# intellerce/controlanimate

Hardware: AMD Instinct MI355X
Metric: frames_per_sec (higher is better)
Workload: dtype fp16

## Files before the change

### controlanimate_amd/_capi.py

```python
from __future__ import annotations

import ctypes as C
import os

_HERE = os.path.dirname(os.path.abspath(__file__))
LIB_PATH = os.environ.get("CA_HIP_LIB") or os.path.join(_HERE, "csrc", "libcontrolanimate_hip.so")

CA_BF16, CA_F16 = 0, 1
CA_F32 = 2
CA_ACT_NONE, CA_ACT_SILU = 0, 1
CA_ACT_RELU = 4
CA_ACT_RELU6 = 5
CA_ACT_LEAKY02 = 6
CA_MLSD_TOPK = 200
CA_POSE_MAX_PEAKS, CA_POSE_MAX_PEOPLE, CA_POSE_AREA_TAPS = 64, 64, 8
CA_POSE_OVERFLOW_PEAKS, CA_POSE_OVERFLOW_PEOPLE = 1, 2
CA_POSE_OVERFLOW_FACES, CA_POSE_OVERFLOW_FACE_RESIZE = 4, 8
CA_FACE_SIZE, CA_FACE_HEAT, CA_FACE_PARTS, CA_FACE_MIN_SIDE, CA_FACE_SLOT_INTS = 384, 48, 71, 11, 8
CA_FACE_MODE_NONE, CA_FACE_MODE_LANCZOS4, CA_FACE_MODE_AREA = 0, 1, 2
CA_POSE_OVERFLOW_HANDS, CA_POSE_OVERFLOW_HAND_RESIZE = 16, 32
CA_HAND_PARTS, CA_HAND_HEAT_COLS, CA_HAND_MAP, CA_HAND_SCALES, CA_HAND_SLOT_INTS = 21, 24, 128, 4, 8
CA_HAND_MODE_NONE, CA_HAND_MODE_RESIZE, CA_HAND_MIN_BOX, CA_HAND_AREA_TAPS = 0, 1, 20, 16
ABI_VERSION = 16


class CAHipUnavailable(RuntimeError):
    pass


class CAHipError(RuntimeError):
    pass


class GemmArgs(C.Structure):
    _fields_ = [
        ("a", C.c_void_p), ("a2", C.c_void_p), ("w", C.c_void_p), ("c", C.c_void_p),
        ("bias", C.c_void_p), ("rowbias", C.c_void_p), ("residual", C.c_void_p),
        ("lda", C.c_int64), ("lda2", C.c_int64), ("ldc", C.c_int64), ("ld_res", C.c_int64),
        ("ld_rowbias", C.c_int64),
        ("m", C.c_int32), ("n", C.c_int32), ("k1", C.c_int32), ("k2", C.c_int32),
        ("rows_per_group", C.c_int32),
        ("alpha", C.c_float), ("post_scale", C.c_float),
        ("act", C.c_int32), ("geglu", C.c_int32), ("out_f32", C.c_int32), ("dtype", C.c_int32),
        ("ln_stats", C.c_void_p), ("ln_colsum", C.c_void_p), ("ln_eps", C.c_float),
        ("workspace", C.c_void_p), ("workspace_bytes", C.c_int64),
        ("row_sums_out", C.c_void_p), ("ln_parts", C.c_int32),
        ("w_frag", C.c_void_p),
    ]


class FfArgs(C.Structure):
    _fields_ = [
        ("x", C.c_void_p), ("w1_frag", C.c_void_p), ("bias1", C.c_void_p), ("colsum1", C.c_void_p), ("ln_stats", C.c_void_p),
        ("w2_frag", C.c_void_p), ("bias2", C.c_void_p), ("residual", C.c_void_p), ("y", C.c_void_p),
        ("lda", C.c_int64), ("ldc", C.c_int64), ("ld_res", C.c_int64),
        ("m", C.c_int32), ("c", C.c_int32), ("inner", C.c_int32), ("ln_eps", C.c_float), ("dtype", C.c_int32),
        ("w_out_frag", C.c_void_p), ("bias_out", C.c_void_p), ("residual_out", C.c_void_p), ("ld_res_out", C.c_int64),
    ]


class TattnArgs(C.Structure):
    _fields_ = [
        ("x", C.c_void_p), ("w_frag", C.c_void_p), ("gamma", C.c_void_p), ("bias_pe", C.c_void_p), ("o", C.c_void_p),
        ("lda", C.c_int64), ("ldo", C.c_int64), ("ld_bias_pe", C.c_int64),
        ("batch", C.c_int32), ("frames", C.c_int32), ("tokens", C.c_int32), ("heads", C.c_int32), ("c", C.c_int32),
        ("ln_eps", C.c_float), ("scale", C.c_float), ("dtype", C.c_int32),
        ("w_out_frag", C.c_void_p), ("bias_out", C.c_void_p), ("residual", C.c_void_p), ("ld_res", C.c_int64),
    ]


ATTN_WOUT_FRAG_ELEMS = 102400
TATTN_W_FRAG_ELEMS = 368640


class XattnArgs(C.Structure):
    _fields_ = [
        ("x", C.c_void_p), ("wq_frag", C.c_void_p), ("bias", C.c_void_p), ("kv_frag", C.c_void_p), ("o", C.c_void_p),
        ("lda", C.c_int64), ("ldo", C.c_int64),
        ("m", C.c_int32), ("tokens", C.c_int32), ("frames_per_kv", C.c_int32), ("kv_mod", C.c_int32), ("kv_batches", C.c_int32),
        ("nk", C.c_int32), ("heads", C.c_int32), ("c", C.c_int32),
        ("ln_eps", C.c_float), ("dtype", C.c_int32),
        ("w_out_frag", C.c_void_p), ("bias_out", C.c_void_p), ("residual", C.c_void_p), ("ld_res", C.c_int64),
        ("kv_frag_ip", C.c_void_p), ("nk_ip", C.c_int32), ("ip_scale", C.c_float),
    ]


XATTN_W_FRAG_ELEMS = 122880
XATTN_KV_FRAG_ELEMS = 7680


class ConvArgs(C.Structure):
    _fields_ = [
        ("x", C.c_void_p), ("x2", C.c_void_p), ("w", C.c_void_p), ("y", C.c_void_p),
        ("bias", C.c_void_p), ("rowbias", C.c_void_p), ("residual", C.c_void_p),
        ("ld_res", C.c_int64), ("ld_rowbias", C.c_int64),
        ("images", C.c_int32), ("hin", C.c_int32), ("win", C.c_int32),
        ("cin1", C.c_int32), ("cin2", C.c_int32), ("cout", C.c_int32),
        ("stride", C.c_int32), ("upsample", C.c_int32), ("rows_per_group", C.c_int32),
        ("alpha", C.c_float), ("post_scale", C.c_float),
        ("act", C.c_int32), ("out_f32", C.c_int32), ("dtype", C.c_int32),
# ... 49 lines not shown
    ]


class PerceiverAttnArgs(C.Structure):
    _fields_ = [
        ("q", C.c_void_p), ("x", C.c_void_p), ("l", C.c_void_p), ("o", C.c_void_p),
        ("q_row", C.c_int64), ("q_batch", C.c_int64),
        ("x_row", C.c_int64), ("x_batch", C.c_int64), ("x_v_off", C.c_int64),
        ("l_row", C.c_int64), ("l_batch", C.c_int64), ("l_v_off", C.c_int64),
        ("o_row", C.c_int64), ("o_batch", C.c_int64),
        ("batches", C.c_int32), ("heads", C.c_int32), ("head_dim", C.c_int32),
        ("nq", C.c_int32), ("n_x", C.c_int32), ("n_l", C.c_int32),
        ("scale", C.c_float), ("dtype", C.c_int32),
    ]


class ModconvArgs(C.Structure):
    _fields_ = [
        ("x", C.c_void_p), ("wt", C.c_void_p), ("s", C.c_void_p), ("demod", C.c_void_p), ("noise", C.c_void_p), ("bias", C.c_void_p),
        ("sft_scale", C.c_void_p), ("sft_shift", C.c_void_p), ("y", C.c_void_p),
        ("s_stride", C.c_int64), ("demod_stride", C.c_int64),
        ("images", C.c_int32), ("h", C.c_int32), ("w", C.c_int32), ("cin", C.c_int32), ("cout", C.c_int32),
        ("upsample", C.c_int32), ("x_shared", C.c_int32),
        ("noise_weight", C.c_float), ("dtype", C.c_int32),
    ]


class Conv7x7Args(C.Structure):
    _fields_ = [
        ("x", C.c_void_p * 2), ("w", C.c_void_p * 2), ("bias", C.c_void_p * 2), ("y", C.c_void_p * 2),
        ("ldx", C.c_int64), ("ldy", C.c_int64),
        ("groups", C.c_int32), ("images", C.c_int32), ("h", C.c_int32), ("w_px", C.c_int32), ("cin", C.c_int32), ("cout", C.c_int32),
        ("relu", C.c_int32), ("dtype", C.c_int32),
    ]


SYMBOLS = {
    "ca_abi_version": (C.c_int, []),
    "ca_last_error": (C.c_char_p, []),
    "ca_gemm": (C.c_int, [C.POINTER(GemmArgs), C.c_void_p]),
    "ca_pack_w_frag": (C.c_int, [C.c_void_p, C.c_int32, C.c_int32, C.c_int32, C.c_void_p, C.c_void_p]),
    "ca_pack_w2_frag": (C.c_int, [C.c_void_p, C.c_int32, C.c_int32, C.c_void_p, C.c_void_p]),
    "ca_ff_fused": (C.c_int, [C.POINTER(FfArgs), C.c_void_p]),
    "ca_ff_fused_supported": (C.c_int, [C.POINTER(FfArgs)]),
    "ca_tattn_fused": (C.c_int, [C.POINTER(TattnArgs), C.c_void_p]),
    "ca_tattn_fused_supported": (C.c_int, [C.POINTER(TattnArgs)]),
    "ca_pack_w_tattn": (C.c_int, [C.c_void_p, C.c_int32, C.c_int32, C.c_void_p, C.c_void_p]),
    "ca_pack_w_out": (C.c_int, [C.c_void_p, C.c_int32, C.c_int32, C.c_void_p, C.c_void_p]),
    "ca_xattn_fused": (C.c_int, [C.POINTER(XattnArgs), C.c_void_p]),
    "ca_xattn_fused_supported": (C.c_int, [C.POINTER(XattnArgs)]),
    "ca_xattn_pack_w": (C.c_int, [C.c_void_p, C.c_int32, C.c_int32, C.c_void_p, C.c_void_p]),
    "ca_xattn_pack_kv": (C.c_int, [C.c_void_p, C.c_int64, C.c_int32, C.c_int32, C.c_int32, C.c_int32, C.c_float, C.c_int32, C.c_void_p, C.c_void_p]),
    "ca_gemm_ln_inline_supported": (C.c_int, [C.POINTER(GemmArgs)]),
    "ca_gemm_wants_finished_stats": (C.c_int, [C.POINTER(GemmArgs)]),
    "ca_ln_finish_sums": (C.c_int, [C.c_void_p, C.c_int, C.c_int64, C.c_int, C.c_float, C.c_void_p, C.c_void_p]),
    "ca_gemm_workspace_bytes": (C.c_int64, [C.POINTER(GemmArgs)]),
    "ca_gemm_row_sums_parts": (C.c_int, [C.POINTER(GemmArgs)]),
    "ca_gemm_plan_name": (C.c_int, [C.POINTER(GemmArgs), C.c_char_p, C.c_int32]),
    "ca_conv3x3_plan_name": (C.c_int, [C.POINTER(ConvArgs), C.c_char_p, C.c_int32]),
    "ca_conv3x3": (C.c_int, [C.POINTER(ConvArgs), C.c_void_p]),
    "ca_pack_w_wino": (C.c_int, [C.c_void_p, C.c_int32, C.c_int32, C.c_int32, C.c_void_p, C.c_void_p]),
    "ca_conv3x3_workspace_bytes": (C.c_int64, [C.POINTER(ConvArgs)]),
    "ca_softmax_rows": (C.c_int, [C.c_void_p, C.c_void_p, C.c_int64, C.c_int32, C.c_int64, C.c_int64, C.c_float, C.c_int32, C.c_void_p]),
    "ca_groupnorm_partials_floats": (C.c_int64, [C.c_int32, C.c_int32, C.c_int32, C.c_int32]),
    "ca_groupnorm_stats": (C.c_int, [C.POINTER(GroupNormArgs), C.c_void_p]),
    "ca_groupnorm_apply": (C.c_int, [C.POINTER(GroupNormArgs), C.c_void_p]),
    "ca_groupnorm": (C.c_int, [C.POINTER(GroupNormArgs), C.c_void_p]),
    "ca_groupnorm_wino_supported": (C.c_int, [C.POINTER(GroupNormArgs)]),
    "ca_layernorm": (C.c_int, [C.POINTER(LayerNormArgs), C.c_void_p]),
    "ca_attention": (C.c_int, [C.POINTER(AttnArgs), C.c_void_p]),
    "ca_attention_plan_name": (C.c_int, [C.POINTER(AttnArgs), C.c_char_p, C.c_int32]),
    "ca_add_bcast": (C.c_int, [C.c_void_p, C.c_void_p, C.c_void_p, C.c_int64, C.c_int64, C.c_int32, C.c_void_p]),
    "ca_repeat": (C.c_int, [C.c_void_p, C.c_void_p, C.c_int64, C.c_int32, C.c_void_p]),
    "ca_silu_f32": (C.c_int, [C.c_void_p, C.c_void_p, C.c_int64, C.c_void_p]),
    "ca_timestep_embedding": (C.c_int, [C.c_void_p, C.c_float, C.c_void_p, C.c_int32, C.c_int32, C.c_int32, C.c_void_p]),
    "ca_latents_to_nhwc": (C.c_int, [C.c_void_p, C.c_void_p, C.c_int32, C.c_int32, C.c_int32, C.c_int32, C.c_int32,
                                      C.c_int32, C.c_int32, C.c_float, C.c_int32, C.c_void_p]),
    "ca_nhwc_to_ncfhw_f32": (C.c_int, [C.c_void_p, C.c_void_p, C.c_int32, C.c_int32, C.c_int32, C.c_int32, C.c_int32,
                                        C.c_int32, C.c_int32, C.c_int32, C.c_void_p]),
    "ca_ncfhw_to_nhwc": (C.c_int, [C.c_void_p, C.c_int32, C.POINTER(C.c_int64), C.c_void_p, C.c_int32, C.c_int32,
                                    C.c_int32, C.c_int32, C.c_int32, C.c_int32, C.c_int32, C.c_void_p]),
    "ca_cfg_scheduler_step": (C.c_int, [C.c_void_p, C.c_int32, C.c_int32, C.c_float, C.c_void_p, C.c_void_p,
                                         C.c_void_p, C.c_void_p, C.c_int32, C.c_int32, C.c_int32, C.c_int32,
                                         C.POINTER(C.c_float), C.c_float, C.c_void_p]),
    "ca_lincomb": (C.c_int, [C.c_void_p, C.POINTER(C.c_void_p), C.POINTER(C.c_float), C.c_int32, C.c_int64, C.c_void_p]),
    "ca_conv3x3_narrow": (C.c_int, [C.POINTER(ConvNarrowArgs), C.c_void_p]),
    "ca_conv3x3_narrow_plan_name": (C.c_int, [C.POINTER(ConvNarrowArgs), C.c_char_p, C.c_int32]),
    "ca_rgb8_to_nhwc": (C.c_int, [C.c_void_p, C.c_void_p, C.c_int32, C.c_int32, C.c_int32, C.c_int32, C.c_void_p]),
    "ca_resize_lanczos4_u8": (C.c_int, [C.c_void_p, C.c_void_p, C.c_int32, C.c_int32, C.c_int32, C.c_int32, C.c_int32,
                                         C.c_void_p, C.c_void_p, C.c_void_p, C.c_void_p, C.c_void_p]),
    "ca_color_match_workspace_bytes": (C.c_int64, [C.c_int32, C.c_int64]),
    "ca_hist_u8x3": (C.c_int, [C.c_void_p, C.c_void_p, C.c_int32, C.c_int64, C.c_void_p]),
    "ca_color_moments_f64": (C.c_int, [C.c_void_p, C.c_void_p, C.c_void_p, C.c_void_p, C.c_int32, C.c_int64, C.c_void_p, C.c_int64, C.c_void_p]),
    "ca_color_transform_f64": (C.c_int, [C.c_void_p, C.c_void_p, C.c_void_p, C.c_void_p, C.c_void_p, C.c_void_p, C.c_int32, C.c_int64, C.c_void_p]),
    "ca_sort_f64_segments": (C.c_int, [C.c_void_p, C.c_void_p, C.c_int32, C.c_int64, C.c_void_p, C.c_int64, C.c_void_p]),
    "ca_color_rank_map_f64": (C.c_int, [C.c_void_p, C.c_void_p, C.c_void_p, C.c_void_p, C.c_void_p, C.c_void_p, C.c_int32, C.c_int64,
                                         C.c_void_p, C.c_int64, C.c_void_p]),
    "ca_color_finish_u8": (C.c_int, [C.c_void_p, C.c_void_p, C.c_int32, C.c_int64, C.c_int32, C.c_void_p, C.c_int64, C.c_void_p]),
    "ca_canny_workspace_bytes": (C.c_int64, [C.c_int32, C.c_int32, C.c_int32]),
    "ca_canny_tile_w": (C.c_int32, []),
    "ca_canny_tile_h": (C.c_int32, []),
    "ca_canny_classify": (C.c_int, [C.c_void_p, C.c_int32, C.c_int32, C.c_int32, C.c_int32, C.c_int32, C.c_int32, C.c_void_p, C.c_int64, C.c_void_p]),
    "ca_canny_link": (C.c_int, [C.c_int32, C.c_int32, C.c_int32, C.c_void_p, C.c_int64, C.c_void_p]),
    "ca_canny_link_stage": (C.c_int, [C.c_int32, C.c_int32, C.c_int32, C.c_void_p, C.c_int64, C.c_int32, C.c_void_p]),
    "ca_canny_emit": (C.c_int, [C.c_int32, C.c_int32, C.c_int32, C.c_void_p, C.c_int64, C.c_void_p, C.c_void_p, C.c_int32, C.c_int32, C.c_void_p]),
    "ca_conv_up2_phase_supported": (C.c_int, [C.POINTER(ConvArgs)]),
# ... 106 lines not shown
```

### controlanimate_amd/context.py

```python
from __future__ import annotations

from dataclasses import dataclass, field
from typing import Optional

import torch


@dataclass
class ExecCtx:
    b: int
    f: int
    dtype: torch.dtype
    temb: torch.Tensor
    emb_groups: int
    ehs: Optional[torch.Tensor] = None
    frames_per_kv: int = 1
    kv_mod: int = 0
    gn_frames_per_stat: int = 1
    cache: dict = field(default_factory=dict)

    @property
    def images(self) -> int:
        return self.b * self.f

    def rows_per_emb_group(self, h: int, w: int) -> int:
        return self.images // self.emb_groups * h * w


class Dispatch:
    gemm_ar = True
    ff_fused = True
    tattn_fused = True
    xattn_fused = True
    attn_out_fused = True
    xattn_ip_fused = True
    conv_winograd = True
    gn_winograd = True
    conv_up2_phase = True
    ln_row_sums = True
    repeat_kernel = True
    ln_fold = True
    cfg_shared = True
    cn_cfg_dedup = True
    pdc_block_fused = True
    dpt_head_fused = False
    pose_conv7_direct = True
    controlnet_streams = 2


dispatch = Dispatch()
```

### controlanimate_amd/controlnet.py

```python
from __future__ import annotations

import dataclasses
from collections import OrderedDict

from typing import List, Optional, Sequence, Tuple, Union

import torch
from torch import nn

from . import kernels as K
from .context import ExecCtx
from .layers import HipConv1x1, HipConv3x3
from .unet import FrozenConfig, HipModelMixin, TimestepEmbedding, Timesteps
from .unet_blocks import UNetMidBlock3DCrossAttn, get_down_block


class ControlNetConditioningEmbedding(nn.Module):
    def __init__(self, conditioning_embedding_channels: int, conditioning_channels: int = 3,
                 block_out_channels: Tuple[int, ...] = (16, 32, 96, 256)):
        super().__init__()
        self.conv_in = HipConv3x3(conditioning_channels, block_out_channels[0])
        blocks = []
        for i in range(len(block_out_channels) - 1):
            blocks.append(HipConv3x3(block_out_channels[i], block_out_channels[i]))
# ... 136 lines not shown
    def residual_scales(self, conditioning_scale: float, guess_mode: bool) -> List[float]:
        n = len(self.controlnet_down_blocks) + 1
        if guess_mode:
            return [float(s) * conditioning_scale for s in torch.logspace(-1, 0, n)]
        return [float(conditioning_scale)] * n

    @torch.no_grad()
    def forward_body(self, x: torch.Tensor, timestep, encoder_hidden_states: torch.Tensor, controlnet_cond: torch.Tensor,
                     conditioning_scale: float = 1.0, guess_mode: bool = False, cfg_identical_halves: bool = False):
        device = x.device
        self._ensure_ready(device)
        images = x.shape[0]
        ehs, cache = self._prompt(encoder_hidden_states, device)
        nb = ehs.shape[0]
        temb = self._time_embedding(timestep, 1, device)
        ctx = ExecCtx(b=images, f=1, dtype=self.act_dtype, temb=temb, emb_groups=1, ehs=ehs, frames_per_kv=1, kv_mod=nb,
                      gn_frames_per_stat=1, cache=cache)
        hint_ent = self._hint(controlnet_cond, device)
        hint = hint_ent["emb"]
        if hint.shape[0] != images:
            raise ValueError(f"controlnet_cond batch {hint.shape[0]} != sample batch {images}")
        first = self.down_blocks[0]
        from .context import dispatch
        same_inputs = (cfg_identical_halves and images % 2 == 0 and bool(hint_ent["doubled"]) and
                       (not torch.is_tensor(timestep) or timestep.numel() == 1))
        if same_inputs and dispatch.cn_cfg_dedup and (images // 2) % nb == 0:
            half = images // 2
            hctx = dataclasses.replace(ctx, b=half)
            x = self.conv_in.run(x[:half], residual=hint[:half])
            outs = [x]
            for blk in self.down_blocks:
                x, o = blk(x, hctx)
                outs += o
            x = self.mid_block(x, hctx)
            return outs, x, self.residual_scales(conditioning_scale, guess_mode), True
        shared = same_inputs and dispatch.cfg_shared and getattr(first, "has_cross_attention", False)
        if shared:
            half = images // 2
            xh = self.conv_in.run(x[:half], residual=hint[:half])
            outs = [K.repeat_batch(xh)]
            x, o = first(xh, ctx, half_ctx=dataclasses.replace(ctx, b=half))
            outs += o
        else:
            x = self.conv_in.run(x, residual=hint)
            outs = [x]
        for blk in (self.down_blocks[1:] if shared else self.down_blocks):
            x, o = blk(x, ctx)
            outs += o
        x = self.mid_block(x, ctx)
        return outs, x, self.residual_scales(conditioning_scale, guess_mode), False

    @torch.no_grad()
    def apply_zero_convs(self, outs, x, scales, accumulate: Optional[Tuple[List[torch.Tensor], torch.Tensor]] = None, twice: bool = False):
        def one(zc, o, scale, prev):
            B_, h, w, c = o.shape
            rows = B_ * h * w
            a = o.view(rows, c)
            if not twice:
                return zc.run(a, alpha=scale, residual=None if prev is None else prev.view(rows, c)).view(B_, h, w, c)
            full = torch.empty((2 * B_, h, w, c), device=o.device, dtype=o.dtype)
            for hf in range(2):
                zc.run(a, alpha=scale, residual=None if prev is None else prev.view(2 * rows, c)[hf * rows:(hf + 1) * rows],
                       out=full.view(2 * rows, c)[hf * rows:(hf + 1) * rows])
            return full
        down = [one(zc, o, scales[i], None if accumulate is None else accumulate[0][i])
                for i, (zc, o) in enumerate(zip(self.controlnet_down_blocks, outs))]
        mid = one(self.controlnet_mid_block, x, scales[-1], None if accumulate is None else accumulate[1])
        return down, mid

    @torch.no_grad()
    def forward_nhwc(self, x: torch.Tensor, timestep, encoder_hidden_states: torch.Tensor, controlnet_cond: torch.Tensor,
                     conditioning_scale: float = 1.0, guess_mode: bool = False,
                     accumulate: Optional[Tuple[List[torch.Tensor], torch.Tensor]] = None, cfg_identical_halves: bool = False):
        outs, xm, scales, twice = self.forward_body(x, timestep, encoder_hidden_states, controlnet_cond, conditioning_scale, guess_mode,
                                                    cfg_identical_halves)
        return self.apply_zero_convs(outs, xm, scales, accumulate, twice)

    def forward(self, sample: torch.Tensor, timestep, encoder_hidden_states: torch.Tensor, controlnet_cond: torch.Tensor,
                conditioning_scale: float = 1.0, class_labels=None, timestep_cond=None, attention_mask=None,
                cross_attention_kwargs=None, guess_mode: bool = False, return_dict: bool = False):
        if not sample.is_cuda:
            raise RuntimeError("ControlNetModel runs on the HIP device only (no CPU fallback)")
        self._ensure_ready(sample.device)
        x = K.ncfhw_to_nhwc(sample.unsqueeze(2), self.conv_in.cin_pad, self.act_dtype)
        down, mid = self.forward_nhwc(x, timestep, encoder_hidden_states, controlnet_cond, conditioning_scale, guess_mode)
        return tuple(d.permute(0, 3, 1, 2) for d in down), mid.permute(0, 3, 1, 2)


class MultiControlNetModel(nn.Module):

    def __init__(self, controlnets: Sequence[ControlNetModel]):
        super().__init__()
        self.nets = nn.ModuleList(controlnets)

    @property
    def dtype(self):
        return self.nets[0].dtype

    def half(self):
        for n in self.nets:
            n.half()
        return self

    def prepare(self, device=None, dtype=None):
        for n in self.nets:
            n.prepare(device, dtype)
        return self

    def forward_bodies(self, x, timestep, encoder_hidden_states, controlnet_cond: Sequence[torch.Tensor],
                       conditioning_scale: Sequence[float], guess_mode: bool = False, cfg_identical_halves: bool = False, streams=None):
        bodies = []
        for i, (net, cond, scale) in enumerate(zip(self.nets, controlnet_cond, conditioning_scale)):
            if streams:
# ... 28 lines not shown
```

### controlanimate_amd/csrc/ca_gemm.hip

```cpp

#include "ca_gemm_plan.h"

namespace {
using namespace ca_gemm_detail;
#include "ca_conv_wino.h"

template <int DT, int BM, int BN, int WAVES_M, int WAVES_N, int MODE>
__global__ __launch_bounds__(256) void k_gemm(GemmKParams p) {
  constexpr int TM = BM / WAVES_M / 16;
  constexpr int TN = BN / WAVES_N / 16;
  constexpr int AI = BM / 32;
  constexpr int BI = BN / 32;
  static_assert(2 * (BM + BN) * BK >= BM * (BN + 8), "epilogue staging must fit");
  __shared__ __attribute__((aligned(16))) u16 smem[2 * (BM + BN) * BK];

  const int tid = threadIdx.x;
  const int lane = tid & 63;
  const int wid = tid >> 6;
  const int wm = wid / WAVES_N, wn = wid % WAVES_N;
  const int g = lane >> 4, l15 = lane & 15;

  const int tiles_n = (p.n + BN - 1) / BN;
  const unsigned bid = xcd_remap(blockIdx.x, gridDim.x);
  int tile_m, tile_n;
// ... 64 lines not shown
    } else {
      const int64_t ld = src2 ? p.lda2 : p.lda;
#pragma unroll
      for (int i = 0; i < AI; ++i) {
        ra[i] = (cok && a_ok[i]) ? ld16(base + a_rowoff[i] * ld + cio) : zero4;
      }
    }
  };
  auto store_tile = [&](int buf) {
    u16* sa = smem + buf * (BM + BN) * BK;
    u16* sb = sa + BM * BK;
#pragma unroll
    for (int i = 0; i < AI; ++i) st16(sa + lds_off(lr + 32 * i, lc), ra[i]);
#pragma unroll
    for (int i = 0; i < BI; ++i) st16(sb + lds_off(lr + 32 * i, lc), rb[i]);
  };

  f32x4 acc[TM][TN];
#pragma unroll
  for (int i = 0; i < TM; ++i)
#pragma unroll
    for (int j = 0; j < TN; ++j) acc[i][j] = (f32x4){0.f, 0.f, 0.f, 0.f};

  const int nt = p.taps * p.kc_tiles;
  load_tile(0);
  store_tile(0);
  __syncthreads();

  for (int t = 0; t < nt; ++t) {
    const int buf = t & 1;
    if (t + 1 < nt) load_tile(t + 1);
    const u16* sa = smem + buf * (BM + BN) * BK;
    const u16* sb = sa + BM * BK;
#pragma unroll
    for (int s = 0; s < 2; ++s) {
      u32x4 fa[TM], fb[TN];
#pragma unroll
      for (int i = 0; i < TM; ++i) fa[i] = ld16(sa + lds_off(wm * TM * 16 + i * 16 + l15, s * 4 + g));
#pragma unroll
      for (int j = 0; j < TN; ++j) fb[j] = ld16(sb + lds_off(wn * TN * 16 + j * 16 + l15, s * 4 + g));
#pragma unroll
      for (int i = 0; i < TM; ++i)
#pragma unroll
        for (int j = 0; j < TN; ++j) acc[i][j] = Elem<DT>::mfma(fb[j], fa[i], acc[i][j]);
    }
    if (t + 1 < nt) store_tile(buf ^ 1);
    __syncthreads();
  }

  gemm_epilogue<DT, BM, BN, TM, TN>(p, acc, smem, m0, n0, wm, wn, l15, g, tid);
}


template <int DT, int BM, int BN, int WAVES_M, int WAVES_N, int MODE, int NBUF>
__global__ __launch_bounds__(256, NBUF == 1 ? (BN > 128 ? 3 : 4) : 2)
void k_gemm_dma(GemmKParams p) {
  static_assert(WAVES_M * WAVES_N == 4 && (NBUF == 1 || NBUF == 3), "instantiations: see above");
  constexpr int KT = BK;
  constexpr int CPR = KT / 8;
  constexpr int RPI = 64 / CPR;
  constexpr int NW = WAVES_M * WAVES_N, NT = NW * 64;
  constexpr int TM = BM / WAVES_M / 16;
  constexpr int TN = BN / WAVES_N / 16;
  constexpr int AG = BM / RPI / NW;
  constexpr int BG = BN / RPI / NW;
  constexpr int SMEM_ELEMS = NBUF * (BM + BN) * KT > BM * (BN + 8) ? NBUF * (BM + BN) * KT : BM * (BN + 8);
  auto swz = [](int row) { return (row >> 1) & 7; };
  auto lds_at = [&](int row, int chunk) { return row * KT + ((chunk ^ swz(row)) << 3); };
  __shared__ __attribute__((aligned(16))) u16 smem[SMEM_ELEMS];

  const int tid = threadIdx.x;
  const int lane = tid & 63;
  const int wid = tid >> 6;
  const int wm = wid / WAVES_N, wn = wid % WAVES_N;
  const int g = lane >> 4, l15 = lane & 15;

  const int tiles_n = (p.n + BN - 1) / BN;
  const int tiles_m = (p.m + BM - 1) / BM;
  unsigned bid = xcd_remap(blockIdx.x, gridDim.x);
  int split = 0;
  if (p.splits > 1) {
    split = bid / (unsigned)(tiles_m * tiles_n);
    bid -= split * (unsigned)(tiles_m * tiles_n);
  }
  int tile_m, tile_n;
  tile_coords(bid, tiles_m, tiles_n, tile_m, tile_n);
  const int m0 = tile_m * BM, n0 = tile_n * BN;

  const __amdgpu_buffer_rsrc_t rs_a = __builtin_amdgcn_make_buffer_rsrc((void*)p.a, 0, p.a_bytes, 0x00020000);
  const __amdgpu_buffer_rsrc_t rs_a2 = __builtin_amdgcn_make_buffer_rsrc((void*)(p.a2 ? p.a2 : p.a), 0, p.a2 ? p.a2_bytes : p.a_bytes, 0x00020000);
  const __amdgpu_buffer_rsrc_t rs_w = __builtin_amdgcn_make_buffer_rsrc((void*)p.w, 0, p.w_bytes, 0x00020000);

  const int r8 = lane / CPR, cp = lane % CPR;
  const int kc = p.c1 + p.c2;
  const int kct = kc / KT;
  const unsigned wld = (unsigned)(p.taps * kc);

  int a_chunk[AG], a_img[AG], a_ho[AG], a_wo[AG];
  unsigned a_off1[AG], a_off2[AG];
  bool a_ok[AG];
#pragma unroll
  for (int i = 0; i < AG; ++i) {
    const int row = (wid * AG + i) * RPI + r8;
    a_chunk[i] = cp ^ swz(row);
    const int m = m0 + row;
    a_ok[i] = m < p.m;
    const int mm = a_ok[i] ? m : p.m - 1;
// ... 78 lines not shown
#pragma unroll
      for (int i = 0; i < TM; ++i) fa[i] = ld16(sa + lds_at(wm * TM * 16 + i * 16 + l15, s * 4 + g));
#pragma unroll
      for (int j = 0; j < TN; ++j) fb[j] = ld16(sb + lds_at(wn * TN * 16 + j * 16 + l15, s * 4 + g));
#pragma unroll
      for (int i = 0; i < TM; ++i)
#pragma unroll
        for (int j = 0; j < TN; ++j) acc[i][j] = Elem<DT>::mfma(fb[j], fa[i], acc[i][j]);
    }
  };
  if (NBUF == 1) {
    for (int t = 0; t < nt; ++t) {
      stage(t_first + t, 0);
      __syncthreads();
      compute(0);
      __syncthreads();
    }
  } else {
    constexpr int PER = AG + BG;
    static_assert((NBUF - 2) * PER < 64, "vmcnt");
#pragma unroll
    for (int s = 0; s < NBUF - 1; ++s)
      if (s < nt) stage(t_first + s, s);
    int slot = 0, slot_in = NBUF - 1;
    for (int t = 0; t < nt; ++t) {
      const int younger = nt - 1 - t < NBUF - 2 ? nt - 1 - t : NBUF - 2;
      if (younger <= 0) asm volatile("s_waitcnt vmcnt(0)" ::: "memory");
      else if (younger == 1) asm volatile("s_waitcnt vmcnt(%0)" ::"n"(PER) : "memory");
      else if (younger == 2) asm volatile("s_waitcnt vmcnt(%0)" ::"n"(2 * PER) : "memory");
      else asm volatile("s_waitcnt vmcnt(%0)" ::"n"((NBUF - 2) * PER < 64 ? (NBUF - 2) * PER : 0) : "memory");
      __builtin_amdgcn_s_barrier();
      if (t + NBUF - 1 < nt) stage(t_first + t + NBUF - 1, slot_in);
      compute(slot);
      asm volatile("s_waitcnt lgkmcnt(0)" ::: "memory");
      slot = slot + 1 == NBUF ? 0 : slot + 1;
      slot_in = slot_in + 1 == NBUF ? 0 : slot_in + 1;
    }
    __syncthreads();
  }
  if (p.splits > 1) {
    float* slab = p.partial + (int64_t)split * p.m * p.n;
#pragma unroll
    for (int i = 0; i < TM; ++i) {
      const int m = m0 + wm * TM * 16 + i * 16 + l15;
      if (m >= p.m) continue;
#pragma unroll
      for (int j = 0; j < TN; ++j) {
        const int n = n0 + wn * TN * 16 + j * 16 + g * 4;
        if (n < p.n) *reinterpret_cast<f32x4*>(slab + (int64_t)m * p.n + n) = acc[i][j];
      }
    }
    return;
  }
  gemm_epilogue<DT, BM, BN, TM, TN, NT>(p, acc, smem, m0, n0, wm, wn, l15, g, tid);
}

template <int DT>
__global__ __launch_bounds__(256) void k_splitk_reduce(GemmKParams p) {
  const int64_t id = (int64_t)blockIdx.x * 256 + threadIdx.x;
  const int c8n = p.n >> 3;
  const int64_t m = id / c8n;
  if (m >= p.m) return;
  const int n = (int)(id - m * c8n) * 8;
  float v[8];
#pragma unroll
  for (int k = 0; k < 8; ++k) v[k] = 0.f;
  for (int sp = 0; sp < p.splits; ++sp) {
    const float* src = p.partial + ((int64_t)sp * p.m + m) * p.n + n;
    const f32x4 a = *reinterpret_cast<const f32x4*>(src), b = *reinterpret_cast<const f32x4*>(src + 4);
#pragma unroll
    for (int k = 0; k < 4; ++k) {
      v[k] += a[k];
      v[4 + k] += b[k];
    }
  }
  if (p.ln_stats) {
    const float2 st = *reinterpret_cast<const float2*>(p.ln_stats + m * 2);
#pragma unroll
    for (int k = 0; k < 8; ++k) v[k] = st.y * (v[k] - st.x * p.ln_colsum[n + k]);
  }
  if (p.bias) {
#pragma unroll
    for (int k = 0; k < 8; ++k) v[k] += p.bias[n + k];
  }
  if (p.rowbias) {
    const float* rbp = p.rowbias + (m / p.rows_per_group) * p.ld_rowbias + n;
#pragma unroll
    for (int k = 0; k < 8; ++k) v[k] += rbp[k];
  }
#pragma unroll
  for (int k = 0; k < 8; ++k) v[k] *= p.alpha;
  unpack8<DT>(pack8<DT>(v), v);
  if (p.res) {
    float r[8];
    unpack8<DT>(ld16(p.res + m * p.ld_res + n), r);
#pragma unroll
    for (int k = 0; k < 8; ++k) v[k] += r[k];
  }
#pragma unroll
  for (int k = 0; k < 8; ++k) v[k] *= p.post;
  if (p.act != CA_ACT_NONE) {
#pragma unroll
    for (int k = 0; k < 8; ++k) v[k] = act_f(v[k], p.act);
  }
  const int64_t off = m * p.ldc + n;
  if (p.out_f32) {
    float* cp = reinterpret_cast<float*>(p.c) + off;
    *reinterpret_cast<f32x4*>(cp) = (f32x4){v[0], v[1], v[2], v[3]};
    *reinterpret_cast<f32x4*>(cp + 4) = (f32x4){v[4], v[5], v[6], v[7]};
  } else {
    st16(reinterpret_cast<u16*>(p.c) + off, pack8<DT>(v));
  }
}

template <int DT, int MODE>
int launch_gemm(const GemmKParams& p, const GemmPlan& g, hipStream_t st) {
  const dim3 grid(ceil_div_i(p.m, g.bm) * ceil_div_i(p.n, g.bn));
  switch (g.kind) {
    case PK_WRES: return ca_launch_gemm_pp(p, DT, MODE, PK_WRES, 0u, st);
    case PK_AR: return ca_launch_gemm_ar(p, DT, st);
    case PK_PP2:
    case PK_PS:
    case PK_PQ: return ca_launch_gemm_pp(p, DT, MODE, g.kind, g.tiles, st);
    case PK_PP2_SPLITK: {
      GemmKParams q = p;
      q.splits = g.splits;
      const int rc = ca_launch_gemm_pp(q, DT, MODE, PK_PP2, g.tiles * (unsigned)g.splits, st);
      hipLaunchKernelGGL((k_splitk_reduce<DT>), dim3(ceil_div_i((int64_t)q.m * (q.n / 8), 256)), dim3(256), 0, st, q);
      return rc;
    }
    case PK_DMA_SPLITK:
      hipLaunchKernelGGL((k_gemm_dma<DT, 128, 128, 2, 2, MODE, 1>), dim3(g.tiles * (unsigned)p.splits), dim3(256), 0, st, p);
      hipLaunchKernelGGL((k_splitk_reduce<DT>), dim3(ceil_div_i((int64_t)p.m * (p.n / 8), 256)), dim3(256), 0, st, p);
      return CA_OK;
    case PK_DMA:
      if (g.bn == 160 && g.nbuf == 1) hipLaunchKernelGGL((k_gemm_dma<DT, 128, 160, 2, 2, MODE, 1>), grid, dim3(256), 0, st, p);
      else if (g.bn == 128 && g.nbuf == 1) hipLaunchKernelGGL((k_gemm_dma<DT, 128, 128, 2, 2, MODE, 1>), grid, dim3(256), 0, st, p);
      else if (g.bn == 64 && g.nbuf == 1) hipLaunchKernelGGL((k_gemm_dma<DT, 128, 64, 4, 1, MODE, 1>), grid, dim3(256), 0, st, p);
      else if (g.bn == 64 && g.nbuf == 3) hipLaunchKernelGGL((k_gemm_dma<DT, 128, 64, 4, 1, MODE, 3>), grid, dim3(256), 0, st, p);
      else break;
      return CA_OK;
    case PK_REG:
      if (g.bn == 128) hipLaunchKernelGGL((k_gemm<DT, 128, 128, 2, 2, MODE>), grid, dim3(256), 0, st, p);
      else if (g.bn == 64) hipLaunchKernelGGL((k_gemm<DT, 128, 64, 4, 1, MODE>), grid, dim3(256), 0, st, p);
      else break;
      return CA_OK;
  }
  CA_FAIL(CA_ERR_LAUNCH, "ca_gemm: no kernel for plan kind %d, tile %dx%d, %d stages", (int)g.kind, g.bm, g.bn, g.nbuf);
}

}

extern "C" int ca_gemm(const ca_gemm_args* a, void* stream) {
  DenseLaunch d;
  int rc = gemm_prepare(a, d);
  if (rc) return rc;
  hipStream_t st = (hipStream_t)stream;
  rc = a->dtype == CA_BF16 ? launch_gemm<CA_BF16, 0>(d.p, d.plan, st) : launch_gemm<CA_F16, 0>(d.p, d.plan, st);
  if (rc) return rc;
  CA_CHECK_LAUNCH("ca_gemm");
  return CA_OK;
}

extern "C" int64_t ca_gemm_workspace_bytes(const ca_gemm_args* a) {
  DenseLaunch d;
  return gemm_resolve(a, d) == CA_OK ? d.workspace : 0;
}

extern "C" int ca_gemm_row_sums_parts(const ca_gemm_args* a) {
  DenseLaunch d;
  DenseAsk ask{};
  ask.without_row_sums = true;
  return gemm_resolve(a, d, ask) == CA_OK ? row_sums_parts_of(d.p) : 0;
}

extern "C" int ca_gemm_ln_inline_supported(const ca_gemm_args* a) {
  DenseLaunch d;
  return a && a->ln_colsum && gemm_resolve(a, d) == CA_OK && wres_eligible(d.p) ? 1 : 0;
}

extern "C" int ca_gemm_wants_finished_stats(const ca_gemm_args* a) {
  if (!a || !a->ln_colsum || !a->ln_stats || a->ln_parts <= 0 || a->row_sums_out) return 0;
  DenseLaunch d;
  DenseAsk ask{};
  ask.stats_finished = true;
  return gemm_resolve(a, d, ask) == CA_OK && d.plan.kind == PK_PQ ? 1 : 0;
}

extern "C" int64_t ca_conv3x3_workspace_bytes(const ca_conv_args* a) { return conv_workspace_bytes(a); }

static int launch_conv_wino(const ca_conv_args* a, const GemmKParams& cp, hipStream_t st) {
  const int kc = a->cin1 + a->cin2;
  const ConvGeom g = conv_geom(a);
  const int64_t tiles = wino_tiles(a, g);
  WinoParams w{};
  w.x = (const u16*)a->x;
  w.x2 = (const u16*)a->x2;
  w.v = (u16*)a->workspace;
  u16* mm = (u16*)a->workspace + (a->x_is_wino_v ? 0 : 16 * tiles * kc);
  w.mm = mm;
  w.y = (u16*)a->y;
  w.bias = a->bias;
  w.rowbias = a->rowbias;
  w.res = (const u16*)a->residual;
  w.ld_res = a->ld_res;
  w.ld_rowbias = a->ld_rowbias;
  w.images = a->images, w.h = g.hl, w.w = g.wl, w.c1 = a->cin1, w.c2 = a->cin2, w.cout = a->cout;
  w.ups = a->upsample;
  w.rows_per_group = cp.rows_per_group;
  w.alpha = a->alpha, w.post = a->post_scale, w.act = a->act;
  const int64_t in_threads = tiles * (kc / 8), out_threads = tiles * (a->cout / 8);
  if (a->x_is_wino_v) w.v = (u16*)a->x;
  else if (a->dtype == CA_BF16) hipLaunchKernelGGL((k_wino_in<CA_BF16>), dim3((unsigned)((in_threads + 255) / 256)), dim3(256), 0, st, w);
  else hipLaunchKernelGGL((k_wino_in<CA_F16>), dim3((unsigned)((in_threads + 255) / 256)), dim3(256), 0, st, w);
  GemmKParams q{};
  q.a = w.v;
  q.w = (const u16*)a->w_wino;
  q.c = mm;
  q.lda = kc;
  q.ldc = a->cout;
  q.a_bytes = desc_bytes(16 * tiles * kc);
  q.w_bytes = desc_bytes((int64_t)16 * a->cout * kc);
  q.m = (int)(16 * tiles);
  q.n = a->cout;
  q.c1 = kc;
  q.taps = 1;
// ... 89 lines not shown
```

### controlanimate_amd/csrc/ca_gemm_core.h

```cpp
#pragma once
#include "ca_common.h"
#include <stdlib.h>

namespace ca_gemm_detail {


struct GemmKParams {
  const u16* a;
  const u16* a2;
  const u16* w;
  void* c;
  const float* bias;
  const float* rowbias;
  const float* ln_stats;
  const float* ln_colsum;
  const u16* res;
  int64_t lda, lda2, ldc, ld_res, ld_rowbias;
  unsigned a_bytes, a2_bytes, w_bytes;
  int m, n;
  int c1, c2;
  int taps;
  int kc_tiles;
  int hin, win, hout, wout, stride, ups, pad_lo;
  int rows_per_group;
  float alpha, post;
  int act, geglu, out_f32;
  int splits;
  float* partial;
  int dbg;
  int tap_inner;
  float* row_sums;
  int ln_parts;
  int ln_inline;
  float ln_eps;
  const u16* wf;
  int w_group_rows;
  unsigned w_group_stride;
  int up2_rows, up2_tiles;
  unsigned up2_mag_w, up2_mag_h;
};

constexpr int BK = 64;

constexpr int GROUP_M = 8;
__device__ __forceinline__ void tile_coords(unsigned bid, int tiles_m, int tiles_n, int& tile_m, int& tile_n) {
  const unsigned gsz = GROUP_M * tiles_n;
  const unsigned group = bid / gsz, in = bid - group * gsz;
  const int first_m = group * GROUP_M;
  const int gm = tiles_m - first_m < GROUP_M ? tiles_m - first_m : GROUP_M;
  tile_m = first_m + in % gm;
  tile_n = in / gm;
}

__device__ __forceinline__ void k_tile_split(const GemmKParams& p, int t, int kct, int& tap, int& cc) {
  if (p.taps == 1) {
    tap = 0;
    cc = t;
  } else if (p.tap_inner) {
    cc = t / p.taps;
    tap = t - cc * p.taps;
  } else {
    tap = t / kct;
    cc = t - tap * kct;
  }
}

__device__ __forceinline__ int lds_off(int row, int chunk) {
  return row * BK + ((chunk ^ ((row >> 1) & 7)) << 3);
}

template <int DT, int TM, int TN>
__device__ __forceinline__ void gemm_epilogue_direct(const GemmKParams& p, f32x4 (&acc)[TM][TN], int m0, int n0, int wm, int wn,
                                                     int l15, int g) {
#pragma unroll
  for (int i = 0; i < TM; ++i) {
    const int m = m0 + wm * TM * 16 + i * 16 + l15;
    if (m >= p.m) continue;
    const float* rbp = p.rowbias ? p.rowbias + (int64_t)(m / p.rows_per_group) * p.ld_rowbias : nullptr;
#pragma unroll
    for (int j = 0; j < TN; ++j) {
      const int n = n0 + wn * TN * 16 + j * 16 + g * 4;
      if (n >= p.n) continue;
      float v[4];
#pragma unroll
      for (int r = 0; r < 4; ++r) v[r] = acc[i][j][r];
      if (p.bias) {
        f32x4 b = *reinterpret_cast<const f32x4*>(p.bias + n);
#pragma unroll
        for (int r = 0; r < 4; ++r) v[r] += b[r];
      }
      if (rbp) {
        f32x4 b = *reinterpret_cast<const f32x4*>(rbp + n);
#pragma unroll
        for (int r = 0; r < 4; ++r) v[r] += b[r];
      }
#pragma unroll
      for (int r = 0; r < 4; ++r) v[r] *= p.alpha;
      if (p.res) {
        u32x2 rr = *reinterpret_cast<const u32x2*>(p.res + (int64_t)m * p.ld_res + n);
        v[0] += Elem<DT>::to_f((u16)(rr[0] & 0xffffu));
        v[1] += Elem<DT>::to_f((u16)(rr[0] >> 16));
        v[2] += Elem<DT>::to_f((u16)(rr[1] & 0xffffu));
        v[3] += Elem<DT>::to_f((u16)(rr[1] >> 16));
      }
#pragma unroll
      for (int r = 0; r < 4; ++r) v[r] *= p.post;
      if (p.act != CA_ACT_NONE) {
#pragma unroll
        for (int r = 0; r < 4; ++r) v[r] = act_f(v[r], p.act);
      }
      if (p.geglu) {
        const f32x2 gg = gelu_erf_f2((f32x2){v[1], v[3]});
        float o0 = v[0] * gg[0];
        float o1 = v[2] * gg[1];
        const int64_t off = (int64_t)m * p.ldc + (n >> 1);
        if (p.out_f32) {
          float* cp = reinterpret_cast<float*>(p.c) + off;
          cp[0] = o0;
          cp[1] = o1;
        } else {
          *reinterpret_cast<unsigned*>(reinterpret_cast<u16*>(p.c) + off) = pack2<DT>(o0, o1);
        }
      } else {
        const int64_t off = (int64_t)m * p.ldc + n;
        if (p.out_f32) {
          *reinterpret_cast<f32x4*>(reinterpret_cast<float*>(p.c) + off) = (f32x4){v[0], v[1], v[2], v[3]};
        } else {
          u32x2 o;
          o[0] = pack2<DT>(v[0], v[1]);
          o[1] = pack2<DT>(v[2], v[3]);
          *reinterpret_cast<u32x2*>(reinterpret_cast<u16*>(p.c) + off) = o;
        }
      }
    }
  }
}

template <int DT, int BM, int BN, int TM, int TN, int NT = 256, bool ROWSUM = false>
__device__ __forceinline__ void gemm_epilogue(const GemmKParams& p, f32x4 (&acc)[TM][TN], u16* cs, int m0, int n0, int wm, int wn,
                                              int l15, int g, int tid, float2* rs = nullptr) {
  if (p.n < 8) {
    gemm_epilogue_direct<DT, TM, TN>(p, acc, m0, n0, wm, wn, l15, g);
    return;
  }
  constexpr int CLD = BN + 8;
  float2 ln_st[TM];
  f32x4 ln_cs[TN];
  if (p.ln_stats) {
#pragma unroll
    for (int i = 0; i < TM; ++i) {
      const int m = m0 + wm * TM * 16 + i * 16 + l15;
      if (p.ln_parts > 0) {
        float a = 0.f, b = 0.f;
        if (m < p.m) {
          for (int q = 0; q < p.ln_parts; ++q) {
            const float2 v = *reinterpret_cast<const float2*>(p.ln_stats + ((int64_t)m * p.ln_parts + q) * 2);
            a += v.x;
            b += v.y;
          }
        }
        const float inv = 1.f / (float)(p.c1 + p.c2);
        const float mean = a * inv;
        ln_st[i] = make_float2(mean, rsqrtf(fmaxf(b * inv - mean * mean, 0.f) + p.ln_eps));
      } else {
        ln_st[i] = m < p.m ? *reinterpret_cast<const float2*>(p.ln_stats + (int64_t)m * 2) : make_float2(0.f, 0.f);
      }
    }
#pragma unroll
    for (int j = 0; j < TN; ++j) {
      const int n = n0 + wn * TN * 16 + j * 16 + g * 4;
      ln_cs[j] = n < p.n ? *reinterpret_cast<const f32x4*>(p.ln_colsum + n) : (f32x4){0.f, 0.f, 0.f, 0.f};
    }
  }
  f32x4 rb_q[TN];
  bool rb_uniform = false;
  if (p.rowbias) {
    const int r_first = m0 + wm * TM * 16, r_last = r_first + TM * 16 - 1;
    rb_uniform = r_last < p.m && r_first / p.rows_per_group == r_last / p.rows_per_group;
    if (rb_uniform) {
      const float* base = p.rowbias + (int64_t)(r_first / p.rows_per_group) * p.ld_rowbias;
#pragma unroll
      for (int j = 0; j < TN; ++j) {
        const int n = n0 + wn * TN * 16 + j * 16 + g * 4;
        rb_q[j] = n < p.n ? *reinterpret_cast<const f32x4*>(base + n) : (f32x4){0.f, 0.f, 0.f, 0.f};
      }
    }
  }
#pragma unroll
  for (int i = 0; i < TM; ++i) {
    const int row = wm * TM * 16 + i * 16 + l15;
    const int m = m0 + row;
    const float* rbp = (p.rowbias && !rb_uniform && m < p.m) ? p.rowbias + (int64_t)(m / p.rows_per_group) * p.ld_rowbias : nullptr;
#pragma unroll
    for (int j = 0; j < TN; ++j) {
      const int col = wn * TN * 16 + j * 16 + g * 4;
      const int n = n0 + col;
      float v[4];
#pragma unroll
      for (int r = 0; r < 4; ++r) v[r] = acc[i][j][r];
      if (n < p.n) {
        if (p.ln_stats) {
#pragma unroll
          for (int r = 0; r < 4; ++r) v[r] = ln_st[i].y * (v[r] - ln_st[i].x * ln_cs[j][r]);
        }
        if (p.bias) {
          const f32x4 b = *reinterpret_cast<const f32x4*>(p.bias + n);
#pragma unroll
          for (int r = 0; r < 4; ++r) v[r] += b[r];
        }
        if (rb_uniform) {
#pragma unroll
          for (int r = 0; r < 4; ++r) v[r] += rb_q[j][r];
        } else if (rbp) {
          const f32x4 b = *reinterpret_cast<const f32x4*>(rbp + n);
#pragma unroll
          for (int r = 0; r < 4; ++r) v[r] += b[r];
        }
      }
      if (p.alpha != 1.f) {
#pragma unroll
        for (int r = 0; r < 4; ++r) v[r] *= p.alpha;
      }
      u32x2 o;
      o[0] = pack2<DT>(v[0], v[1]);
      o[1] = pack2<DT>(v[2], v[3]);
      *reinterpret_cast<u32x2*>(cs + row * CLD + col) = o;
    }
  }
  __syncthreads();
  constexpr int CH = BN / 8;
  const bool simple = p.post == 1.f && p.act == CA_ACT_NONE && !p.geglu && !p.out_f32;
  const bool geglu_only = p.geglu && p.post == 1.f && p.act == CA_ACT_NONE && !p.res && !p.out_f32;
#pragma unroll
  for (int u = 0; u < BM * CH / NT; ++u) {
    const int id = tid + u * NT;
    const int row = id / CH, c8 = id - row * CH;
    const int m = m0 + row, n = n0 + c8 * 8;
    if (m >= p.m || n >= p.n) continue;
    if (simple) {
      u32x4 pk = ld16(cs + row * CLD + c8 * 8);
      if (p.res) {
        const u32x4 rr = ld16(p.res + (int64_t)m * p.ld_res + n);
        if (DT == CA_F16) {
#pragma unroll
          for (int k = 0; k < 4; ++k) {
            unsigned s_;
            asm("v_pk_add_f16 %0, %1, %2" : "=v"(s_) : "v"(pk[k]), "v"(rr[k]));
            pk[k] = s_;
          }
        } else {
          float a_[8], r_[8];
          unpack8<DT>(pk, a_);
          unpack8<DT>(rr, r_);
#pragma unroll
          for (int k = 0; k < 8; ++k) a_[k] += r_[k];
          pk = pack8<DT>(a_);
        }
      }
      st16(reinterpret_cast<u16*>(p.c) + (int64_t)m * p.ldc + n, pk);
      if (ROWSUM && p.row_sums) {
        float r[8];
        unpack8<DT>(pk, r);
        float a = 0.f, b = 0.f;
#pragma unroll
        for (int k = 0; k < 8; ++k) {
          a += r[k];
          b = fmaf(r[k], r[k], b);
        }
        rs[row * CH + c8] = make_float2(a, b);
      }
      continue;
    }
    if (geglu_only) {
      float v[8];
      unpack8<DT>(ld16(cs + row * CLD + c8 * 8), v);
      const f32x2 g0 = gelu_erf_f2((f32x2){v[1], v[3]}), g1 = gelu_erf_f2((f32x2){v[5], v[7]});
      u32x2 w;
      w[0] = pack2<DT>(v[0] * g0[0], v[2] * g0[1]);
      w[1] = pack2<DT>(v[4] * g1[0], v[6] * g1[1]);
      *reinterpret_cast<u32x2*>(reinterpret_cast<u16*>(p.c) + (int64_t)m * p.ldc + (n >> 1)) = w;
      continue;
    }
    float v[8];
    unpack8<DT>(ld16(cs + row * CLD + c8 * 8), v);
    if (p.res) {
      float r[8];
      unpack8<DT>(ld16(p.res + (int64_t)m * p.ld_res + n), r);
#pragma unroll
      for (int k = 0; k < 8; ++k) v[k] += r[k];
    }
#pragma unroll
    for (int k = 0; k < 8; ++k) v[k] *= p.post;
    if (p.act != CA_ACT_NONE) {
#pragma unroll
      for (int k = 0; k < 8; ++k) v[k] = act_f(v[k], p.act);
    }
    if (p.geglu) {
      float o[4];
#pragma unroll
      for (int k = 0; k < 4; k += 2) {
        const f32x2 gg = gelu_erf_f2((f32x2){v[2 * k + 1], v[2 * k + 3]});
        o[k] = v[2 * k] * gg[0];
        o[k + 1] = v[2 * k + 2] * gg[1];
      }
      const int64_t off = (int64_t)m * p.ldc + (n >> 1);
      if (p.out_f32) {
        *reinterpret_cast<f32x4*>(reinterpret_cast<float*>(p.c) + off) = (f32x4){o[0], o[1], o[2], o[3]};
      } else {
        u32x2 w;
        w[0] = pack2<DT>(o[0], o[1]);
        w[1] = pack2<DT>(o[2], o[3]);
        *reinterpret_cast<u32x2*>(reinterpret_cast<u16*>(p.c) + off) = w;
      }
    } else {
      const int64_t off = (int64_t)m * p.ldc + n;
      if (p.out_f32) {
        float* cp = reinterpret_cast<float*>(p.c) + off;
        *reinterpret_cast<f32x4*>(cp) = (f32x4){v[0], v[1], v[2], v[3]};
        *reinterpret_cast<f32x4*>(cp + 4) = (f32x4){v[4], v[5], v[6], v[7]};
      } else {
        const u32x4 pk = pack8<DT>(v);
        st16(reinterpret_cast<u16*>(p.c) + off, pk);
        if (ROWSUM && p.row_sums) {
          float r[8];
          unpack8<DT>(pk, r);
          float a = 0.f, b = 0.f;
#pragma unroll
          for (int k = 0; k < 8; ++k) {
            a += r[k];
            b = fmaf(r[k], r[k], b);
          }
          rs[row * CH + c8] = make_float2(a, b);
        }
      }
    }
  }
  if (ROWSUM && p.row_sums) {
    __syncthreads();
    if (tid < BM && m0 + tid < p.m) {
      float a = 0.f, b = 0.f;
      for (int c8 = 0; c8 < CH; ++c8) {
        const float2 v = rs[tid * CH + c8];
        a += v.x;
        b += v.y;
      }
      *reinterpret_cast<float2*>(p.row_sums + ((int64_t)(m0 + tid) * (p.n / BN) + n0 / BN) * 2) = make_float2(a, b);
    }
  }
}


constexpr unsigned DMA_OOB = 0xFFFFFFF0u;

enum PlanKind {
  PK_WRES = 0,
  PK_PP2,
  PK_PP2_SPLITK,
  PK_DMA,
  PK_DMA_SPLITK,
  PK_REG,
  PK_PS,
  PK_PQ,
  PK_AR,
};

constexpr int64_t FIT31 = 0x7FFFFF00ll;
inline int64_t out_rows(const GemmKParams& p) { return p.up2_rows ? 4 * (int64_t)p.up2_rows : (int64_t)p.m; }
inline int64_t c_extent_bytes(const GemmKParams& p) { return ((out_rows(p) - 1) * p.ldc + (p.geglu ? p.n / 2 : p.n)) * 2; }
inline int64_t res_extent_bytes(const GemmKParams& p) { return p.res ? ((out_rows(p) - 1) * p.ld_res + p.n) * 2 : 0; }
inline bool act_out_fit31(const GemmKParams& p) {
  return c_extent_bytes(p) < FIT31 && res_extent_bytes(p) < FIT31 && p.a_bytes < FIT31 && (!p.c2 || p.a2_bytes < FIT31);
}

}

int ca_launch_gemm_pp(const ca_gemm_detail::GemmKParams& p, int dtype, int mode, ca_gemm_detail::PlanKind kind, unsigned tiles, hipStream_t st);
int ca_launch_gemm_ar(const ca_gemm_detail::GemmKParams& p, int dtype, hipStream_t st);
```

### controlanimate_amd/csrc/ca_gemm_plan.h

```cpp
#pragma once
#include "ca_gemm_core.h"

namespace ca_gemm_detail {

inline unsigned desc_bytes(int64_t elems) {
  const int64_t b = elems * 2;
  return (b > 0 && b < (int64_t)0xFFFFFF00ll) ? (unsigned)b : 0u;
}

inline bool dma_shape_ok(const GemmKParams& p) { return (p.c1 + p.c2) % BK == 0 && (p.c2 == 0 || p.c1 % BK == 0); }
inline bool dma_sizes_ok(const GemmKParams& p) { return p.a_bytes != 0 && p.w_bytes != 0 && (p.c2 == 0 || p.a2_bytes != 0); }
inline bool dma_capable(const GemmKParams& p) { return dma_shape_ok(p) && dma_sizes_ok(p); }

inline bool wres_eligible(const GemmKParams& p) {
  static const int wres_env = CA_KNOB("CA_GEMM_WRES", -1);
  const int kc = p.c1 + p.c2;
  return wres_env != 0 && kc == 320 && p.taps == 1 && (p.c2 == 0 || p.c1 % 32 == 0) && p.n % 160 == 0 && p.n / 160 <= 32 && !p.out_f32 &&
         p.splits <= 1 && !p.ln_parts && dma_sizes_ok(p) &&
         (!p.rowbias || p.rows_per_group % 32 == 0) &&
         act_out_fit31(p) &&
         (wres_env == 1 || p.m >= 16384);
}

inline bool ar_eligible(const GemmKParams& p, bool scratch) {
// ... 126 lines not shown

inline int check_epilogue(const char* who, int n, int geglu, int64_t ldc, int64_t ld_res, const void* res) {
  CA_REQUIRE(n == 4 || (n >= 8 && n % 8 == 0), "%s: N=%d must be 4 or a multiple of 8", who, n);
  CA_REQUIRE(!geglu || n % 8 == 0, "%s: geglu needs N %% 8 == 0", who);
  if (n >= 8) {
    CA_REQUIRE(ldc % (geglu ? 4 : 8) == 0, "%s: ldc=%lld must be a multiple of %d", who, (long long)ldc, geglu ? 4 : 8);
    CA_REQUIRE(!res || ld_res % 8 == 0, "%s: ld_res=%lld must be a multiple of 8", who, (long long)ld_res);
  } else {
    CA_REQUIRE(ldc % 4 == 0, "%s: ldc=%lld misaligned", who, (long long)ldc);
    CA_REQUIRE(!res || ld_res % 4 == 0, "%s: ld_res=%lld misaligned", who, (long long)ld_res);
  }
  return CA_OK;
}

struct DenseAsk {
  bool without_row_sums;
  bool stats_finished;
};

inline int gemm_fill(const ca_gemm_args* a, GemmKParams& p, const DenseAsk& ask) {
  CA_REQUIRE(a != nullptr, "ca_gemm: null args");
  CA_REQUIRE(a->a && a->w && a->c, "ca_gemm: null operand");
  CA_REQUIRE(a->m > 0 && a->k1 > 0 && a->k2 >= 0, "ca_gemm: bad sizes m=%d k1=%d k2=%d", a->m, a->k1, a->k2);
  CA_REQUIRE(a->k1 % 8 == 0 && a->k2 % 8 == 0, "ca_gemm: k1=%d k2=%d must be multiples of 8", a->k1, a->k2);
  CA_REQUIRE(a->lda % 8 == 0 && (a->k2 == 0 || (a->a2 && a->lda2 % 8 == 0)), "ca_gemm: lda/lda2 misaligned or a2 missing");
  CA_REQUIRE(a->dtype == CA_BF16 || a->dtype == CA_F16, "ca_gemm: dtype %d", a->dtype);
  CA_REQUIRE(!a->rowbias || a->rows_per_group > 0, "ca_gemm: rows_per_group");
  CA_REQUIRE(!a->rowbias || a->ld_rowbias % 4 == 0, "ca_gemm: ld_rowbias misaligned");
  int rc = check_epilogue("ca_gemm", a->n, a->geglu, a->ldc, a->ld_res, a->residual);
  if (rc) return rc;
  p.a = (const u16*)a->a, p.a2 = (const u16*)a->a2, p.w = (const u16*)a->w, p.c = a->c;
  p.bias = a->bias, p.rowbias = a->rowbias, p.ln_stats = a->ln_stats, p.ln_colsum = a->ln_colsum;
  p.row_sums = ask.without_row_sums ? nullptr : a->row_sums_out;
  p.ln_parts = ask.stats_finished ? 0 : a->ln_parts;
  CA_REQUIRE(p.ln_parts >= 0 && p.ln_parts <= 16, "ca_gemm: ln_parts=%d", p.ln_parts);
  CA_REQUIRE(p.ln_parts == 0 || (a->ln_stats && a->ln_colsum && a->ln_eps > 0.f), "ca_gemm: ln_parts needs ln_stats (the partial sums), ln_colsum and ln_eps > 0");
  p.ln_inline = (a->ln_colsum && !a->ln_stats) ? 1 : 0;
  p.ln_eps = a->ln_eps;
  p.wf = (const u16*)a->w_frag;
  CA_REQUIRE(!a->ln_stats || a->ln_colsum, "ca_gemm: ln_stats without ln_colsum");
  CA_REQUIRE(!p.ln_inline || a->ln_eps > 0.f, "ca_gemm: ln_colsum without ln_stats asks for in-kernel statistics and needs ln_eps > 0");
  CA_REQUIRE(!a->ln_colsum || (a->n >= 8 && a->k2 == 0), "ca_gemm: the folded LayerNorm needs N >= 8 and a single A source");
  p.res = (const u16*)a->residual;
  p.lda = a->lda, p.lda2 = a->lda2, p.ldc = a->ldc, p.ld_res = a->ld_res, p.ld_rowbias = a->ld_rowbias;
  p.a_bytes = desc_bytes((int64_t)(a->m - 1) * a->lda + a->k1);
  p.a2_bytes = a->k2 ? desc_bytes((int64_t)(a->m - 1) * a->lda2 + a->k2) : 0u;
  p.w_bytes = desc_bytes((int64_t)a->n * (a->k1 + a->k2));
  p.m = a->m, p.n = a->n, p.c1 = a->k1, p.c2 = a->k2;
  p.taps = 1;
  p.kc_tiles = ceil_div_i(a->k1 + a->k2, BK);
  p.rows_per_group = a->rows_per_group > 0 ? a->rows_per_group : 1;
  p.alpha = a->alpha, p.post = a->post_scale, p.act = a->act, p.geglu = a->geglu, p.out_f32 = a->out_f32;
  p.splits = 1;
  return CA_OK;
}

struct DenseLaunch {
  GemmKParams p;
  GemmPlan plan;
  int64_t workspace;
};
inline int gemm_resolve(const ca_gemm_args* a, DenseLaunch& d, const DenseAsk& ask = DenseAsk{}) {
  d = DenseLaunch{};
  GemmKParams& p = d.p;
  int rc = gemm_fill(a, p, ask);
  if (rc) return rc;
  const SplitK k = splitk_decide(p, 0);
  splitk_apply(k, a->workspace, a->workspace_bytes, p);
  d.workspace = k.bytes;
  if (p.ln_inline && p.wf) {
    if (ar_eligible(p, true)) d.workspace = (int64_t)p.m * 8;
    if (a->workspace && a->workspace_bytes >= (int64_t)p.m * 8) p.partial = reinterpret_cast<float*>(a->workspace);
  }
  d.plan = plan_gemm(p, 0);
  return CA_OK;
}

inline int gemm_prepare(const ca_gemm_args* a, DenseLaunch& d) {
  int rc = gemm_resolve(a, d);
  if (rc) return rc;
  CA_REQUIRE(!d.p.row_sums || row_sums_capable(d.p), "ca_gemm: row_sums_out is not available for this launch: ask ca_gemm_row_sums_parts() first");
  CA_REQUIRE(!d.p.ln_inline || wres_eligible(d.p), "ca_gemm: in-kernel LayerNorm statistics (ln_stats NULL) are not available for this launch: "
             "ask ca_gemm_ln_inline_supported() first and pass ln_stats otherwise");
  return CA_OK;
}

struct ConvGeom { int hl, wl, hout, wout; int64_t m; };
inline ConvGeom conv_geom(const ca_conv_args* a) {
  ConvGeom g;
  g.hl = a->hin << a->upsample, g.wl = a->win << a->upsample;
  const int pad = a->pad_asym ? 1 : 2;
  g.hout = (g.hl + pad - 3) / a->stride + 1;
  g.wout = (g.wl + pad - 3) / a->stride + 1;
  g.m = (int64_t)a->images * g.hout * g.wout;
  return g;
}
inline int64_t wino_tiles(const ca_conv_args* a, const ConvGeom& g) { return (int64_t)a->images * (g.hl / 2) * (g.wl / 2); }

inline int64_t wino_workspace_bytes(const ca_conv_args* a) {
  if (!a || !a->w_wino || (a->dtype != CA_F16 && a->dtype != CA_BF16) || a->stride != 1 || a->pad_asym || a->out_f32) return 0;
  if (a->upsample != 0 && a->upsample != 1) return 0;
  if (a->x_is_wino_v && (a->cin2 != 0 || a->upsample)) return 0;
  const ConvGeom g = conv_geom(a);
  if (a->images <= 0 || g.hl < 2 || g.wl < 2 || (g.hl & 1) || (g.wl & 1)) return 0;
  const int kc = a->cin1 + a->cin2;
  static const int min_cin = CA_KNOB("CA_WINO_MIN_CIN", 1280);
  if (kc < 640 || kc % BK != 0 || a->cin1 % 8 != 0 || a->cin2 % 8 != 0 || a->cout % 320 != 0) return 0;
  const int64_t tiles = wino_tiles(a, g);
  if (kc < min_cin && !(min_cin == 1280 && tiles <= 4096)) return 0;
  static const int max_tiles = CA_KNOB("CA_WINO_MAX_TILES", 16384);
  if (tiles % 256 != 0 || tiles > max_tiles) return 0;
  if (16 * tiles * (int64_t)(kc > a->cout ? kc : a->cout) * 2 >= 0x7FFFFF00ll) return 0;
  return 16 * tiles * (int64_t)((a->x_is_wino_v ? 0 : kc) + a->cout) * 2;
}

inline bool wino_taken(const ca_conv_args* a) {
  const int64_t wb = wino_workspace_bytes(a);
  return wb > 0 && a->workspace && a->workspace_bytes >= wb && (((uintptr_t)a->workspace | (uintptr_t)a->w_wino) & 15) == 0;
}

inline void conv_fill_sizes(const ca_conv_args* a, const ConvGeom& g, GemmKParams& p) {
  p.a_bytes = desc_bytes((int64_t)a->images * a->hin * a->win * a->cin1);
  p.a2_bytes = a->cin2 ? desc_bytes((int64_t)a->images * a->hin * a->win * a->cin2) : 0u;
  p.w_bytes = desc_bytes((int64_t)a->cout * 9 * (a->cin1 + a->cin2));
  p.m = (int)g.m, p.n = a->cout, p.c1 = a->cin1, p.c2 = a->cin2;
  p.taps = 9;
  static const int tap_inner_env = CA_KNOB("CA_CONV_TAP_INNER", 1);
  p.tap_inner = tap_inner_env;
  p.kc_tiles = ceil_div_i(a->cin1 + a->cin2, BK);
  p.hin = a->hin, p.win = a->win, p.hout = g.hout, p.wout = g.wout;
  p.stride = a->stride, p.ups = a->upsample, p.pad_lo = a->pad_asym ? 0 : 1;
  p.geglu = 0, p.out_f32 = a->out_f32;
  p.splits = 1;
}

inline int conv_prepare(const ca_conv_args* a, GemmKParams& p) {
// ... 81 lines not shown
```

### controlanimate_amd/csrc/ca_gemm_pp.hip

```cpp
#include "ca_gemm_core.h"
#include <type_traits>

namespace {
using namespace ca_gemm_detail;
#include "ca_gemm_pp2.h"
#include "ca_gemm_wres.h"
#include "ca_gemm_ps.h"
#include "ca_gemm_pq.h"

int cu_count() {
  static int n = 0;
  if (!n) {
    int dev = 0;
    hipDeviceProp_t prop;
    if (hipGetDevice(&dev) == hipSuccess && hipGetDeviceProperties(&prop, dev) == hipSuccess) n = prop.multiProcessorCount;
    if (n <= 0) n = 256;
  }
  return n;
}

template <class Launch>
int launch_stamped(const GemmKParams& p, hipStream_t st, const char* label, unsigned sep, unsigned eol, Launch launch) {
  static unsigned long long* dbuf = nullptr;
  if (!dbuf && hipMalloc(&dbuf, 4096 * 8) != hipSuccess) return CA_ERR_LAUNCH;
  (void)hipMemsetAsync(dbuf, 0, 4096 * 8, st);
  GemmKParams q = p;
  q.partial = reinterpret_cast<float*>(dbuf);
  launch(q);
  (void)hipStreamSynchronize(st);
  static int printed = 0;
  if (printed++ < 1) {
    static unsigned long long host[4096];
    (void)hipMemcpy(host, dbuf, sizeof(host), hipMemcpyDeviceToHost);
    for (int g = 0; g < 2; ++g) {
      fprintf(stderr, "[%s stamps group %d, %dx%dx%d] tag:delta_cycles ...\n", label, g, p.m, p.n, (p.c1 + p.c2) * p.taps);
      unsigned long long prev = host[g * 2048];
      for (int i = 0; i < 1000 && host[g * 2048 + 2 * i]; ++i) {
        fprintf(stderr, "%llu:%llu ", host[g * 2048 + 2 * i + 1], host[g * 2048 + 2 * i] - prev);
        prev = host[g * 2048 + 2 * i];
        if (host[g * 2048 + 2 * i + 1] == sep) fprintf(stderr, "| ");
        if (host[g * 2048 + 2 * i + 1] == eol) fprintf(stderr, "\n");
      }
      fprintf(stderr, "\n");
    }
  }
  return CA_OK;
}

template <int DT, int MODE>
int launch_pp(const GemmKParams& p, PlanKind kind, unsigned tiles, hipStream_t st) {
  const unsigned c_bytes = (unsigned)c_extent_bytes(p), res_bytes = (unsigned)res_extent_bytes(p);
  const unsigned grid = tiles < (unsigned)cu_count() ? tiles : (unsigned)cu_count();
  switch (kind) {
    case PK_PQ: {
      auto launch = [&](const GemmKParams& q) {
        if (MODE == 0 && (q.geglu || q.ln_colsum || q.ln_stats)) hipLaunchKernelGGL((k_gemm_pq<DT, 0, 1>), dim3(grid), dim3(512), 0, st, q, (int)tiles, c_bytes, 0u);
        else if (MODE == 0 && q.row_sums) hipLaunchKernelGGL((k_gemm_pq<DT, 0, 2>), dim3(grid), dim3(512), 0, st, q, (int)tiles, c_bytes, res_bytes);
        else hipLaunchKernelGGL((k_gemm_pq<DT, MODE>), dim3(grid), dim3(512), 0, st, q, (int)tiles, c_bytes, res_bytes);
      };
#ifdef CA_STAMPS
      if (p.dbg == 9) return launch_stamped(p, st, "pq", 8, 10, launch);
#endif
      launch(p);
      return CA_OK;
    }
    case PK_PS: {
      auto launch = [&](const GemmKParams& q) { hipLaunchKernelGGL((k_gemm_ps<DT, MODE>), dim3(grid), dim3(512), 0, st, q, (int)tiles, c_bytes, res_bytes); };
#ifdef CA_STAMPS
      if (p.dbg == 9) return launch_stamped(p, st, "ps", 8, 10, launch);
#endif
      launch(p);
      return CA_OK;
    }
    case PK_WRES: {
      if (MODE != 0) return CA_ERR_LAUNCH;
      const int panels = p.n / 160;
      const int chunks = (p.m + 255) / 256;
      int per = (cu_count() / 8) / panels;
      if (per * 8 > chunks) per = chunks / 8;
      if (per < 1) per = 1;
      const unsigned rb_bytes = p.rowbias ? (unsigned)(((int64_t)((p.m - 1) / p.rows_per_group) * p.ld_rowbias + p.n) * 4) : 16u;
      hipLaunchKernelGGL((k_gemm_wres<DT>), dim3(8 * per * panels), dim3(512), 0, st, p, panels, 8 * per, chunks, rb_bytes, c_bytes, res_bytes);
      return CA_OK;
    }
    case PK_PP2:
      hipLaunchKernelGGL((k_gemm_pp2<DT, MODE>), dim3(tiles), dim3(512), 0, st, p);
      return CA_OK;
    default: return CA_ERR_LAUNCH;
  }
}

template <int DT>
int launch_up2(const GemmKParams& p, PlanKind kind, unsigned tiles, hipStream_t st) {
  if (kind != PK_PQ) return CA_ERR_LAUNCH;
  const unsigned grid = tiles < (unsigned)cu_count() ? tiles : (unsigned)cu_count();
  hipLaunchKernelGGL((k_gemm_pq<DT, 2>), dim3(grid), dim3(512), 0, st, p, (int)tiles, (unsigned)c_extent_bytes(p), (unsigned)res_extent_bytes(p));
  return CA_OK;
}
}

int ca_launch_gemm_pp(const ca_gemm_detail::GemmKParams& p0, int dtype, int mode, ca_gemm_detail::PlanKind kind, unsigned tiles, hipStream_t st) {
  static const int dbg = CA_KNOB("CA_PP_DBG", 0);
  ca_gemm_detail::GemmKParams p = p0;
  p.dbg = dbg;
  if (mode == 2) return dtype == CA_BF16 ? launch_up2<CA_BF16>(p, kind, tiles, st) : launch_up2<CA_F16>(p, kind, tiles, st);
  if (dtype == CA_BF16) return mode ? launch_pp<CA_BF16, 1>(p, kind, tiles, st) : launch_pp<CA_BF16, 0>(p, kind, tiles, st);
  return mode ? launch_pp<CA_F16, 1>(p, kind, tiles, st) : launch_pp<CA_F16, 0>(p, kind, tiles, st);
}
```

### controlanimate_amd/csrc/ca_gemm_pp2.h

```cpp
template <int DT, int MODE>
__global__ __launch_bounds__(512, 2) void k_gemm_pp2(GemmKParams p) {
  constexpr int BM = 128, BN = 320, KT = 64;
  constexpr int TM = 4, TN = 5;
  constexpr int A_ROWS = 128, B0_ROWS = 128, B1_ROWS = 192;
  constexpr int OFF_A = 0, OFF_B0 = A_ROWS * KT, OFF_B1 = (A_ROWS + B0_ROWS) * KT;
  constexpr int BUF = (A_ROWS + B0_ROWS + B1_ROWS) * KT;
  constexpr int RS_ELEMS = BM * (BN / 8) * 4;
  constexpr int SMEM_ELEMS = 2 * BUF > BM * (BN + 8) + RS_ELEMS ? 2 * BUF : BM * (BN + 8) + RS_ELEMS;
  __shared__ __attribute__((aligned(16))) u16 smem[SMEM_ELEMS];

  const int tid = threadIdx.x;
  const int lane = tid & 63;
  const int wid = tid >> 6;
  const int wr = wid >> 2, wc = wid & 3;
  const int g = lane >> 4, l15 = lane & 15;

  const int tiles_n = p.n / BN;
  const int tiles_m = (p.m + BM - 1) / BM;
  unsigned bid = xcd_remap(blockIdx.x, gridDim.x);
  int split = 0;
  if (p.splits > 1) {
    split = bid / (unsigned)(tiles_m * tiles_n);
    bid -= split * (unsigned)(tiles_m * tiles_n);
  }
  int tile_m, tile_n;
  tile_coords(bid, tiles_m, tiles_n, tile_m, tile_n);
  const int m0 = tile_m * BM, n0 = tile_n * BN;

  const __amdgpu_buffer_rsrc_t rs_a = __builtin_amdgcn_make_buffer_rsrc((void*)p.a, 0, p.a_bytes, 0x00020000);
  const __amdgpu_buffer_rsrc_t rs_a2 = __builtin_amdgcn_make_buffer_rsrc((void*)(p.a2 ? p.a2 : p.a), 0, p.a2 ? p.a2_bytes : p.a_bytes, 0x00020000);
  const __amdgpu_buffer_rsrc_t rs_w = __builtin_amdgcn_make_buffer_rsrc((void*)p.w, 0, p.w_bytes, 0x00020000);

  auto swz = [](int row) { return (row >> 1) & 7; };
  const int r8 = lane >> 3, cp = lane & 7;
  const int kc = p.c1 + p.c2;
  const int kct = kc / KT;
  const unsigned wld = (unsigned)(p.taps * kc);

  int a_chunk[2], a_img[2], a_ho[2], a_wo[2];
  unsigned a_off1[2], a_off2[2];
  bool a_ok[2];
#pragma unroll
  for (int i = 0; i < 2; ++i) {
    const int r = (wid * 2 + i) * 8 + r8;
    a_chunk[i] = cp ^ swz(r);
    const int m = m0 + r;
    a_ok[i] = m < p.m;
    const int mm = a_ok[i] ? m : p.m - 1;
    if (MODE == 1) {
      const int hw = p.hout * p.wout;
      a_img[i] = mm / hw;
      const int rem = mm - a_img[i] * hw;
      a_ho[i] = rem / p.wout;
// ... 118 lines not shown
    if (t + 1 < nt) asm volatile("s_waitcnt vmcnt(7)" ::: "memory");
    else asm volatile("s_waitcnt vmcnt(0)" ::: "memory");
    __builtin_amdgcn_s_barrier();
    __builtin_amdgcn_sched_barrier(0);
    __builtin_amdgcn_s_setprio(1);
#pragma unroll
    for (int s = 0; s < 2; ++s)
#pragma unroll
      for (int i = 0; i < 4; ++i)
#pragma unroll
        for (int j = 0; j < 2; ++j) acc[i][j] = Elem<DT>::mfma(fb0[j][s], fa[i][s], acc[i][j]);
    __builtin_amdgcn_s_setprio(0);
    __builtin_amdgcn_sched_barrier(0);
    __builtin_amdgcn_s_barrier();
#pragma unroll
    for (int s = 0; s < 2; ++s)
#pragma unroll
      for (int j = 0; j < 3; ++j) fb1[j][s] = ld16(buf + fb1_off[j][s]);
    issue_ab0(t + 2);
    asm volatile("s_waitcnt lgkmcnt(0)" ::: "memory");
    if (t + 2 < nt) asm volatile("s_waitcnt vmcnt(7)" ::: "memory");
    else if (t + 1 < nt) asm volatile("s_waitcnt vmcnt(3)" ::: "memory");
    else asm volatile("s_waitcnt vmcnt(0)" ::: "memory");
    __builtin_amdgcn_s_barrier();
    __builtin_amdgcn_sched_barrier(0);
    __builtin_amdgcn_s_setprio(1);
#pragma unroll
    for (int s = 0; s < 2; ++s)
#pragma unroll
      for (int i = 0; i < 4; ++i)
#pragma unroll
        for (int j = 0; j < 3; ++j) acc[i][2 + j] = Elem<DT>::mfma(fb1[j][s], fa[i][s], acc[i][2 + j]);
    __builtin_amdgcn_s_setprio(0);
    __builtin_amdgcn_sched_barrier(0);
    __builtin_amdgcn_s_barrier();
  }
  if (wr == 0) __builtin_amdgcn_s_barrier();
  __syncthreads();
  if (p.dbg == 1) {
    if (acc[0][0][0] == 12345.678f) *reinterpret_cast<float*>(p.c) = acc[3][1][2] + acc[2][TN - 1][1];
    return;
  }
  if (p.splits > 1) {
    float* slab = p.partial + (int64_t)split * p.m * p.n;
#pragma unroll
    for (int i = 0; i < TM; ++i) {
      const int m = m0 + wr * 64 + i * 16 + l15;
      if (m >= p.m) continue;
#pragma unroll
      for (int j = 0; j < TN; ++j) *reinterpret_cast<f32x4*>(slab + (int64_t)m * p.n + n0 + wc * 80 + j * 16 + g * 4) = acc[i][j];
    }
    return;
  }
  gemm_epilogue<DT, BM, BN, TM, TN, 512, true>(p, acc, smem, m0, n0, wr, wc, l15, g, tid, reinterpret_cast<float2*>(smem + BM * (BN + 8)));
}
```

### controlanimate_amd/csrc/ca_gemm_ps.h

```cpp

#include "ca_gemm_seq.h"

__device__ __forceinline__ void ca_ps_vm_wait(int n) {
  n = __builtin_amdgcn_readfirstlane(n > 23 ? 23 : (n < 0 ? 0 : n));
  asm volatile(
      "s_cmp_ge_i32 %0, 12\n\ts_cbranch_scc1 30f\n\t"
      "s_cmp_ge_i32 %0, 6\n\ts_cbranch_scc1 31f\n\t"
      "s_cmp_ge_i32 %0, 3\n\ts_cbranch_scc1 32f\n\t"
      "s_cmp_ge_i32 %0, 1\n\ts_cbranch_scc1 33f\n\t"
      "s_waitcnt vmcnt(0)\n\ts_branch 99f\n"
      "33:\n\ts_cmp_ge_i32 %0, 2\n\ts_cbranch_scc1 34f\n\ts_waitcnt vmcnt(1)\n\ts_branch 99f\n"
      "34:\n\ts_waitcnt vmcnt(2)\n\ts_branch 99f\n"
      "32:\n\ts_cmp_ge_i32 %0, 4\n\ts_cbranch_scc1 35f\n\ts_waitcnt vmcnt(3)\n\ts_branch 99f\n"
      "35:\n\ts_cmp_ge_i32 %0, 5\n\ts_cbranch_scc1 36f\n\ts_waitcnt vmcnt(4)\n\ts_branch 99f\n"
      "36:\n\ts_waitcnt vmcnt(5)\n\ts_branch 99f\n"
      "31:\n\ts_cmp_ge_i32 %0, 9\n\ts_cbranch_scc1 37f\n\ts_cmp_ge_i32 %0, 7\n\ts_cbranch_scc1 38f\n\ts_waitcnt vmcnt(6)\n\ts_branch 99f\n"
      "38:\n\ts_cmp_ge_i32 %0, 8\n\ts_cbranch_scc1 39f\n\ts_waitcnt vmcnt(7)\n\ts_branch 99f\n"
      "39:\n\ts_waitcnt vmcnt(8)\n\ts_branch 99f\n"
      "37:\n\ts_cmp_ge_i32 %0, 10\n\ts_cbranch_scc1 40f\n\ts_waitcnt vmcnt(9)\n\ts_branch 99f\n"
      "40:\n\ts_cmp_ge_i32 %0, 11\n\ts_cbranch_scc1 41f\n\ts_waitcnt vmcnt(10)\n\ts_branch 99f\n"
      "41:\n\ts_waitcnt vmcnt(11)\n\ts_branch 99f\n"
      "30:\n\ts_cmp_ge_i32 %0, 18\n\ts_cbranch_scc1 42f\n\ts_cmp_ge_i32 %0, 15\n\ts_cbranch_scc1 43f\n"
      "s_cmp_ge_i32 %0, 13\n\ts_cbranch_scc1 44f\n\ts_waitcnt vmcnt(12)\n\ts_branch 99f\n"
      "44:\n\ts_cmp_ge_i32 %0, 14\n\ts_cbranch_scc1 45f\n\ts_waitcnt vmcnt(13)\n\ts_branch 99f\n"
      "45:\n\ts_waitcnt vmcnt(14)\n\ts_branch 99f\n"
      "43:\n\ts_cmp_ge_i32 %0, 16\n\ts_cbranch_scc1 46f\n\ts_waitcnt vmcnt(15)\n\ts_branch 99f\n"
      "46:\n\ts_cmp_ge_i32 %0, 17\n\ts_cbranch_scc1 47f\n\ts_waitcnt vmcnt(16)\n\ts_branch 99f\n"
      "47:\n\ts_waitcnt vmcnt(17)\n\ts_branch 99f\n"
      "42:\n\ts_cmp_ge_i32 %0, 21\n\ts_cbranch_scc1 48f\n\ts_cmp_ge_i32 %0, 19\n\ts_cbranch_scc1 49f\n\ts_waitcnt vmcnt(18)\n\ts_branch 99f\n"
      "49:\n\ts_cmp_ge_i32 %0, 20\n\ts_cbranch_scc1 50f\n\ts_waitcnt vmcnt(19)\n\ts_branch 99f\n"
      "50:\n\ts_waitcnt vmcnt(20)\n\ts_branch 99f\n"
      "48:\n\ts_cmp_ge_i32 %0, 22\n\ts_cbranch_scc1 51f\n\ts_waitcnt vmcnt(21)\n\ts_branch 99f\n"
      "51:\n\ts_cmp_ge_i32 %0, 23\n\ts_cbranch_scc1 52f\n\ts_waitcnt vmcnt(22)\n\ts_branch 99f\n"
      "52:\n\ts_waitcnt vmcnt(23)\n"
      "99:\n"
      :
      : "s"(n)
      : "scc", "memory");
}

__device__ __forceinline__ int ca_ps_col(int j, int i, bool geglu) {
  if (j == 4) return 64 + i;
  if (geglu) return 16 * (i >> 2) + 4 * j + (i & 3);
  return 32 * (j >> 1) + 8 * (i >> 2) + 4 * (j & 1) + (i & 3);
}

template <int DT, int MODE>
__global__ __launch_bounds__(512, 2) void k_gemm_ps(GemmKParams p, int tiles_total, unsigned c_bytes, unsigned res_bytes) {
  constexpr int BM = 128, BN = 320, KT = 64;
  constexpr int TM = 4, TN = 5;
  constexpr int A_ROWS = 128, B0_ROWS = 128, B1_ROWS = 192;
  constexpr int OFF_A = 0, OFF_B0 = A_ROWS * KT, OFF_B1 = (A_ROWS + B0_ROWS) * KT;
  constexpr int BUF = (A_ROWS + B0_ROWS + B1_ROWS) * KT;
  constexpr int PAR_BASE = 2 * BUF * 2;
  constexpr int P_CS = 0, P_BI = 2048, P_RB0 = 4096, P_RB1 = 6144, P_ST = 8192, PSET = 12288;
  constexpr int FLAG_BASE = PAR_BASE + 2 * PSET;
  constexpr int RS_BASE = FLAG_BASE + 8 * 4 * 256;
  constexpr int SMEM_BYTES = RS_BASE + 128 * 4 * 8;
  static_assert(SMEM_BYTES <= 160 * 1024, "LDS");
  __shared__ __attribute__((aligned(16))) unsigned char smem_b[SMEM_BYTES];
  u16* const smem = reinterpret_cast<u16*>(smem_b);

  const int tid = threadIdx.x;
  const int lane = tid & 63;
  const int wid = __builtin_amdgcn_readfirstlane(tid >> 6);
  const int wr = wid >> 2, wc = wid & 3;
  const int g = lane >> 4, l15 = lane & 15;

  const int tiles_n = p.n / BN;
  const int tiles_m = (p.m + BM - 1) / BM;
  const int G = gridDim.x;
  const int bslot = (G % 8 == 0) ? (int)(blockIdx.x % 8) * (G / 8) + (int)(blockIdx.x / 8) : (int)blockIdx.x;
  const int my_tiles = bslot < tiles_total ? (tiles_total - bslot + G - 1) / G : 0;
  if (my_tiles == 0) return;

  for (int i = tid; i < 8 * 4 * 64; i += 512) reinterpret_cast<unsigned*>(smem_b + FLAG_BASE)[i] = 0xFFFFFFFFu;
  __syncthreads();

  const __amdgpu_buffer_rsrc_t rs_a = __builtin_amdgcn_make_buffer_rsrc((void*)p.a, 0, p.a_bytes, 0x00020000);
  const __amdgpu_buffer_rsrc_t rs_a2 = __builtin_amdgcn_make_buffer_rsrc((void*)(p.a2 ? p.a2 : p.a), 0, p.a2 ? p.a2_bytes : p.a_bytes, 0x00020000);
  const __amdgpu_buffer_rsrc_t rs_w = __builtin_amdgcn_make_buffer_rsrc((void*)p.w, 0, p.w_bytes, 0x00020000);
  const __amdgpu_buffer_rsrc_t rs_c = __builtin_amdgcn_make_buffer_rsrc(p.c, 0, c_bytes, 0x00020000);
  const __amdgpu_buffer_rsrc_t rs_cs = __builtin_amdgcn_make_buffer_rsrc((void*)(p.ln_colsum ? (const void*)p.ln_colsum : (const void*)p.w), 0, p.ln_colsum ? (unsigned)p.n * 4u : 0u, 0x00020000);
  const __amdgpu_buffer_rsrc_t rs_bi = __builtin_amdgcn_make_buffer_rsrc((void*)(p.bias ? (const void*)p.bias : (const void*)p.w), 0, p.bias ? (unsigned)p.n * 4u : 0u, 0x00020000);
  const unsigned st_row_bytes = p.ln_parts > 0 ? (unsigned)p.ln_parts * 8u : 8u;
  const __amdgpu_buffer_rsrc_t rs_st = __builtin_amdgcn_make_buffer_rsrc((void*)(p.ln_stats ? (const void*)p.ln_stats : (const void*)p.w), 0, p.ln_stats ? (unsigned)p.m * st_row_bytes : 0u, 0x00020000);
  const unsigned long long res_addr = (unsigned long long)(p.res ? (const void*)p.res : (const void*)p.c);
  const u32x4 rs_res = {(unsigned)__builtin_amdgcn_readfirstlane((int)(unsigned)res_addr), (unsigned)__builtin_amdgcn_readfirstlane((int)(unsigned)((res_addr >> 32) & 0xffffu)),
                        (unsigned)__builtin_amdgcn_readfirstlane((int)(p.res ? res_bytes : 0u)), 0x00020000u};
  const unsigned rb_groups = p.rowbias ? (unsigned)((p.m + p.rows_per_group - 1) / p.rows_per_group) : 0u;
  const __amdgpu_buffer_rsrc_t rs_rb = __builtin_amdgcn_make_buffer_rsrc((void*)(p.rowbias ? (const void*)p.rowbias : (const void*)p.w), 0,
                                                                         p.rowbias ? (unsigned)(((int64_t)(rb_groups - 1) * p.ld_rowbias + p.n) * 4) : 0u, 0x00020000);
  const __amdgpu_buffer_rsrc_t rs_seq = __builtin_amdgcn_make_buffer_rsrc((void*)ca_seq_table.v, 0, 4096u, 0x00020000);

#ifdef CA_STAMPS
  unsigned long long* const stamps = reinterpret_cast<unsigned long long*>(p.partial);
  int stamp_i = 0;
  auto stamp = [&](int tag) __attribute__((always_inline)) {
    if (p.dbg == 9 && blockIdx.x == 0 && (wid == 0 || wid == 4) && lane == 0 && stamp_i < 1000) {
      stamps[(wid >> 2) * 2048 + 2 * stamp_i] = __builtin_readcyclecounter();
// ... 151 lines not shown
      d_c0 += KT;
    } else if (++d_tap == p.taps) {
      d_tap = 0;
      d_c0 += KT;
    }
  };

  auto flag_begin = [&](int slot) __attribute__((always_inline)) -> unsigned {
    unsigned fv;
    const unsigned addr = (unsigned)(size_t)(__attribute__((address_space(3))) unsigned char*)(my_flags + slot * 256);
    asm volatile("ds_read_b32 %0, %1" : "=v"(fv) : "v"(addr) : "memory");
    return fv;
  };
  auto flag_finish = [&](int slot, int seqno, unsigned fv) __attribute__((always_inline)) {
    asm volatile("s_waitcnt lgkmcnt(0)" : "+v"(fv)::"memory");
    const unsigned want = (unsigned)(seqno & 1023);
    if ((unsigned)__builtin_amdgcn_readfirstlane(fv) == want) return;
    const unsigned addr = (unsigned)(size_t)(__attribute__((address_space(3))) unsigned char*)(my_flags + slot * 256);
    for (unsigned spins = 0; spins < (1u << 20); ++spins) {
      __builtin_amdgcn_s_sleep(1);
      unsigned v;
      asm volatile("ds_read_b32 %0, %1\n\ts_waitcnt lgkmcnt(0)" : "=v"(v) : "v"(addr) : "memory");
      if ((unsigned)__builtin_amdgcn_readfirstlane(v) == want) return;
    }
    asm volatile("s_waitcnt vmcnt(0)" ::: "memory");
  };

  f32x4 acc[TM][TN];
#pragma unroll
  for (int i = 0; i < TM; ++i)
#pragma unroll
    for (int j = 0; j < TN; ++j) acc[i][j] = (f32x4){0.f, 0.f, 0.f, 0.f};

  int fa_base[2], fb0_base[2], fb1_base[2];
  {
    const int ra = wr * 64 + l15, rb0 = wc * 32 + l15, rb1 = wc * 48 + l15;
    fa_base[0] = OFF_A + ra * KT + ((g ^ swz(ra)) << 3);
    fb0_base[0] = OFF_B0 + rb0 * KT + ((g ^ swz(rb0)) << 3);
    fb1_base[0] = OFF_B1 + rb1 * KT + ((g ^ swz(rb1)) << 3);
    fa_base[1] = fa_base[0] ^ 32;
    fb0_base[1] = fb0_base[0] ^ 32;
    fb1_base[1] = fb1_base[0] ^ 32;
  }
  u32x4 fa[4][2], fb0[2][2], fb1[3][2];

  u32x4 res16[TM][2];
  u32x2 res8[TM];
#pragma unroll
  for (int i = 0; i < TM; ++i) {
    res16[i][0] = res16[i][1] = (u32x4){0u, 0u, 0u, 0u};
    res8[i] = (u32x2){0u, 0u};
  }
  int mark_res = 0;
  auto res_prefetch = [&](int m0, int n0) __attribute__((always_inline)) {
    int lane_o = lane;
    asm volatile("" : "+v"(lane_o));
    const int l15o = lane_o & 15, go = lane_o >> 4;
#pragma unroll
    for (int i = 0; i < TM; ++i) {
      const int m = m0 + wr * 64 + i * 16 + l15o;
      const unsigned rowoff = m < p.m ? (unsigned)m * (unsigned)p.ld_res * 2u + (unsigned)(n0 + wc * 80) * 2u : OOB_V;
      const unsigned o0 = rowoff + (unsigned)(8 * go) * 2u, o1 = rowoff + (unsigned)(32 + 8 * go) * 2u, o2 = rowoff + (unsigned)(64 + 4 * go) * 2u;
      asm volatile("s_nop 4\n\tbuffer_load_dwordx4 %0, %3, %6, 0 offen\n\tbuffer_load_dwordx4 %1, %4, %6, 0 offen\n\tbuffer_load_dwordx2 %2, %5, %6, 0 offen"
                   : "=&v"(res16[i][0]), "=&v"(res16[i][1]), "=&v"(res8[i])
                   : "v"(o0), "v"(o1), "v"(o2), "s"(rs_res)
                   : "memory");
    }
    issued += 3 * TM;
    mark_res = issued;
  };
  auto res_wait = [&]() __attribute__((always_inline)) {
    ca_ps_vm_wait(issued - mark_res);
    asm volatile("" : "+v"(res16[0][0]), "+v"(res16[0][1]), "+v"(res16[1][0]), "+v"(res16[1][1]), "+v"(res16[2][0]), "+v"(res16[2][1]), "+v"(res16[3][0]), "+v"(res16[3][1])::"memory");
    asm volatile("" : "+v"(res8[0]), "+v"(res8[1]), "+v"(res8[2]), "+v"(res8[3])::"memory");
  };

  auto mfma_p1 = [&]() __attribute__((always_inline)) {
    __builtin_amdgcn_sched_barrier(0);
    __builtin_amdgcn_s_setprio(1);
#pragma unroll
    for (int s = 0; s < 2; ++s)
#pragma unroll
      for (int i = 0; i < 4; ++i)
#pragma unroll
        for (int j = 0; j < 2; ++j) acc[i][j] = Elem<DT>::mfma(fb0[j][s], fa[i][s], acc[i][j]);
    __builtin_amdgcn_s_setprio(0);
    __builtin_amdgcn_sched_barrier(0);
  };
  auto mfma_p2 = [&]() __attribute__((always_inline)) {
    __builtin_amdgcn_sched_barrier(0);
    __builtin_amdgcn_s_setprio(1);
#pragma unroll
    for (int s = 0; s < 2; ++s)
#pragma unroll
      for (int i = 0; i < 4; ++i)
#pragma unroll
        for (int j = 0; j < 3; ++j) acc[i][2 + j] = Elem<DT>::mfma(fb1[j][s], fa[i][s], acc[i][2 + j]);
    __builtin_amdgcn_s_setprio(0);
    __builtin_amdgcn_sched_barrier(0);
  };

  bool rs_pending = false;
  int rs_m0 = 0, rs_tn = 0;
  auto rs_flush = [&]() __attribute__((always_inline)) {
    if (!rs_pending) return;
    rs_pending = false;
    if (wc != 0) return;
    int lane_o = lane;
    asm volatile("" : "+v"(lane_o));
    const int row = wr * 64 + lane_o, m = rs_m0 + row;
    const f32x4 q0 = *reinterpret_cast<const f32x4*>(smem_b + RS_BASE + row * 32), q1 = *reinterpret_cast<const f32x4*>(smem_b + RS_BASE + row * 32 + 16);
    const float a = (((0.f + q0[0]) + q0[2]) + q1[0]) + q1[2], b = (((0.f + q0[1]) + q0[3]) + q1[1]) + q1[3];
    if (m < p.m) *reinterpret_cast<float2*>(p.row_sums + ((int64_t)m * tiles_n + rs_tn) * 2) = make_float2(a, b);
  };
// ... 20 lines not shown
          } else {
            const f32x4 v = *reinterpret_cast<const f32x4*>(pset + P_ST + row * 32), w = *reinterpret_cast<const f32x4*>(pset + P_ST + row * 32 + 16);
            a = (((0.f + v[0]) + v[2]) + w[0]) + w[2];
            b = (((0.f + v[1]) + v[3]) + w[1]) + w[3];
          }
          const float mean = a * inv;
          st[i] = make_float2(mean, rsqrtf(fmaxf(b * inv - mean * mean, 0.f) + p.ln_eps));
        }
      } else {
        u32x2 s0, s1, s2, s3;
        const unsigned addr = (unsigned)(size_t)(__attribute__((address_space(3))) const unsigned char*)(pset + P_ST + (wr * 64 + l15) * 8);
        asm volatile("ds_read_b64 %0, %4\n\tds_read_b64 %1, %4 offset:128\n\tds_read_b64 %2, %4 offset:256\n\tds_read_b64 %3, %4 offset:384\n\ts_waitcnt lgkmcnt(0)"
                     : "=&v"(s0), "=&v"(s1), "=&v"(s2), "=&v"(s3) : "v"(addr) : "memory");
        const u32x2 sv[TM] = {s0, s1, s2, s3};
#pragma unroll
        for (int i = 0; i < TM; ++i) {
          const float x = __uint_as_float(sv[i][0]), y = __uint_as_float(sv[i][1]);
          if (p.ln_parts == 1) {
            const float mean = (0.f + x) * inv;
            st[i] = make_float2(mean, rsqrtf(fmaxf((0.f + y) * inv - mean * mean, 0.f) + p.ln_eps));
          } else {
            st[i] = make_float2(x, y);
          }
        }
      }
    }
    if (!p.ln_stats) {
#pragma unroll
      for (int i = 0; i < TM; ++i) st[i] = make_float2(0.f, 1.f);
    }
    int rb_sel = 0;
    if (p.rowbias) rb_sel = (m0 + wr * 64) / p.rows_per_group - m0 / p.rows_per_group;
    const unsigned char* rbp = pset + (rb_sel ? P_RB1 : P_RB0);
    unsigned rowoff[TM];
#pragma unroll
    for (int i = 0; i < TM; ++i) {
      const int m = m0 + wr * 64 + i * 16 + l15;
      rowoff[i] = (m < p.m && p.dbg != 1) ? (unsigned)m * (unsigned)p.ldc * 2u + (unsigned)((geglu ? (n0 >> 1) + wc * 40 : n0 + wc * 80)) * 2u : OOB_V;
    }
    float rsum[TM], rsq[TM];
#pragma unroll
    for (int i = 0; i < TM; ++i) rsum[i] = rsq[i] = 0.f;

    struct Par {
      f32x4 cs, bi, rb;
    };
    auto load_par = [&](int c0) __attribute__((always_inline)) -> Par {
      Par q;
      q.cs = *reinterpret_cast<const f32x4*>(pset + P_CS + c0 * 4);
      q.bi = *reinterpret_cast<const f32x4*>(pset + P_BI + c0 * 4);
      q.rb = *reinterpret_cast<const f32x4*>(rbp + c0 * 4);
      return q;
    };
    auto staged = [&](int i, int j, const Par& q, float (&v)[4]) __attribute__((always_inline)) {
#pragma unroll
      for (int r = 0; r < 4; ++r) {
        float x = st[i].y * (acc[i][j][r] - st[i].x * q.cs[r]);
        x = (x + q.bi[r]) + q.rb[r];
        v[r] = x * p.alpha;
      }
      acc[i][j] = (f32x4){0.f, 0.f, 0.f, 0.f};
    };

    if (p.res) res_wait();
    if (!geglu) {
#pragma unroll
      for (int pr = 0; pr < 3; ++pr) {
        const int nq = pr < 2 ? 2 : 1;
        Par par[2];
#pragma unroll
        for (int u = 0; u < 2; ++u)
          if (u < nq) par[u] = load_par(wc * 80 + (pr < 2 ? 32 * pr + 8 * g + 4 * u : 64 + 4 * g));
#pragma unroll
        for (int i = 0; i < TM; ++i) {
          unsigned w[4] = {0u, 0u, 0u, 0u};
#pragma unroll
          for (int u = 0; u < 2; ++u) {
            if (u >= nq) break;
            float v[4];
            staged(i, pr * 2 + u, par[u], v);
            w[2 * u] = pack2<DT>(v[0], v[1]);
            w[2 * u + 1] = pack2<DT>(v[2], v[3]);
          }
#pragma unroll
          for (int k = 0; k < 4; ++k) {
            if (k >= 2 * nq) break;
            const unsigned rr = pr < 2 ? res16[i][pr & 1][k] : res8[i][k & 1];
            if (DT == CA_F16) {
              unsigned s_;
              asm("v_pk_add_f16 %0, %1, %2" : "=v"(s_) : "v"(w[k]), "v"(rr));
              w[k] = s_;
            } else {
              w[k] = pack2<DT>(Elem<DT>::to_f((u16)(w[k] & 0xffffu)) + Elem<DT>::to_f((u16)(rr & 0xffffu)),
                               Elem<DT>::to_f((u16)(w[k] >> 16)) + Elem<DT>::to_f((u16)(rr >> 16)));
            }
          }
          if (p.row_sums) {
#pragma unroll
            for (int k = 0; k < 4; ++k) {
              if (k >= 2 * nq) break;
              const float lo = Elem<DT>::to_f((u16)(w[k] & 0xffffu)), hi = Elem<DT>::to_f((u16)(w[k] >> 16));
              rsum[i] += lo + hi;
              rsq[i] = fmaf(lo, lo, fmaf(hi, hi, rsq[i]));
            }
          }
          if (pr < 2) __builtin_amdgcn_raw_buffer_store_b128((u32x4){w[0], w[1], w[2], w[3]}, rs_c, rowoff[i] + (unsigned)(32 * pr + 8 * g) * 2u, 0, 0);
          else __builtin_amdgcn_raw_buffer_store_b64((u32x2){w[0], w[1]}, rs_c, rowoff[i] + (unsigned)(64 + 4 * g) * 2u, 0, 0);
        }
      }
      issued += 3 * TM;
    } else {
      Par par[TN];
#pragma unroll
      for (int j = 0; j < TN; ++j) par[j] = load_par(wc * 80 + (j < 4 ? 16 * g + 4 * j : 64 + 4 * g));
#pragma unroll
      for (int i = 0; i < TM; ++i) {
        unsigned w[TN];
#pragma unroll
        for (int j = 0; j < TN; ++j) {
          float v[4];
          staged(i, j, par[j], v);
#pragma unroll
          for (int r = 0; r < 4; ++r) v[r] = Elem<DT>::to_f(Elem<DT>::from_f(v[r]));
          const f32x2 gg = gelu_erf_f2((f32x2){v[1], v[3]});
          w[j] = pack2<DT>(v[0] * gg[0], v[2] * gg[1]);
        }
        __builtin_amdgcn_raw_buffer_store_b128((u32x4){w[0], w[1], w[2], w[3]}, rs_c, rowoff[i] + (unsigned)(8 * g) * 2u, 0, 0);
        __builtin_amdgcn_raw_buffer_store_b32(w[4], rs_c, rowoff[i] + (unsigned)(32 + 2 * g) * 2u, 0, 0);
      }
      issued += 2 * TM;
    }
    if (p.row_sums) {
#pragma unroll
      for (int i = 0; i < TM; ++i) {
        float a = rsum[i], b = rsq[i];
        a += __shfl_xor(a, 16);
        b += __shfl_xor(b, 16);
        a += __shfl_xor(a, 32);
        b += __shfl_xor(b, 32);
        if (g == 0) {
          const unsigned addr = (unsigned)(size_t)(__attribute__((address_space(3))) unsigned char*)(smem_b + RS_BASE + (wr * 64 + i * 16 + l15) * 32 + wc * 8);
          const u32x2 ab = {__float_as_uint(a), __float_as_uint(b)};
          asm volatile("ds_write_b64 %0, %1" ::"v"(addr), "v"(ab) : "memory");
        }
      }
      rs_pending = true;
      rs_m0 = m0;
      rs_tn = tn;
    }
    asm volatile("s_waitcnt lgkmcnt(0)" ::: "memory");
  };

#define CA_PS_SET_TILE(SEQ)                                    \
  {                                                            \
    int tm_, tn_;                                              \
    d_live = tile_of((SEQ), tm_, tn_);                         \
    if (d_live) dma_set_tile((SEQ), tm_ * BM, tn_ * BN);       \
  }
  CA_PS_SET_TILE(0)
  issue_ab0();
// ... 77 lines not shown
```

### controlanimate_amd/csrc/ca_gemm_wres.h

```cpp
#include "ca_gemm_seq.h"

__device__ __forceinline__ int ca_wres_col(int j, int i, bool geglu) {
  if (geglu) return 16 * j + i;
  return 32 * (j >> 1) + 8 * (i >> 2) + 4 * (j & 1) + (i & 3);
}

template <int DT>
__global__ __launch_bounds__(512, 1) void k_gemm_wres(GemmKParams p, int panels, int lanes, int chunks, unsigned rb_bytes, unsigned c_bytes, unsigned res_bytes) {
  constexpr int K = 320, PN = 160, TN = 10, KQ = 10;
  constexpr int WLD_B = 656;
  constexpr int W_BYTES = PN * WLD_B;
  constexpr int SLOT = 2048, RING = 3 * SLOT;
  constexpr int OFF_PAR = W_BYTES + 8 * RING;
  constexpr int OFF_RB = OFF_PAR + 1280;
  constexpr int OFF_FLAG = OFF_RB + 8 * 1024;
  __shared__ __attribute__((aligned(16))) unsigned char smem[OFF_FLAG + 8 * 16];
  static_assert(OFF_FLAG + 8 * 16 <= 160 * 1024, "LDS");

  const int tid = threadIdx.x;
  const int lane = tid & 63;
  const int wid = __builtin_amdgcn_readfirstlane(tid >> 6);
  const int g = lane >> 4, l15 = lane & 15;

  const int slot_b = blockIdx.x >> 3;
  const int panel = slot_b % panels;
  const int my_lane = (blockIdx.x & 7) + 8 * (slot_b / panels);
  if (my_lane >= lanes) return;
  const int n0 = panel * PN;

  const bool geglu = p.geglu != 0;
  for (int q = tid; q < PN * (K / 8); q += 512) {
    const int row = q / (K / 8), c = q - row * (K / 8);
    *reinterpret_cast<u32x4*>(smem + row * WLD_B + c * 16) = ld16(p.w + (int64_t)(n0 + ca_wres_col(row >> 4, row & 15, geglu)) * K + c * 8);
  }
  if (tid < 2 * PN) {
    const float* src = tid < PN ? p.bias : p.ln_colsum;
    const int n = tid < PN ? tid : tid - PN;
    reinterpret_cast<float*>(smem + OFF_PAR)[tid] = src ? src[n0 + n] : 0.f;
  }
  __syncthreads();

  const __amdgpu_buffer_rsrc_t rs_rb = __builtin_amdgcn_make_buffer_rsrc((void*)(p.rowbias ? (const void*)p.rowbias : (const void*)p.w), 0, rb_bytes, 0x00020000);
  unsigned char* rb_patch = smem + OFF_RB + wid * 1024;
  const __amdgpu_buffer_rsrc_t rs_c = __builtin_amdgcn_make_buffer_rsrc(p.c, 0, c_bytes, 0x00020000);
  const __amdgpu_buffer_rsrc_t rs_res = __builtin_amdgcn_make_buffer_rsrc((void*)(p.res ? (const void*)p.res : (const void*)p.c), 0, p.res ? res_bytes : 0u, 0x00020000);
  const __amdgpu_buffer_rsrc_t rs_a = __builtin_amdgcn_make_buffer_rsrc((void*)p.a, 0, p.a_bytes, 0x00020000);
  const __amdgpu_buffer_rsrc_t rs_a2 = __builtin_amdgcn_make_buffer_rsrc((void*)(p.a2 ? p.a2 : p.a), 0, p.a2 ? p.a2_bytes : p.a_bytes, 0x00020000);
  unsigned char* ring = smem + W_BYTES + wid * RING;
  const __amdgpu_buffer_rsrc_t rs_seq = __builtin_amdgcn_make_buffer_rsrc((void*)ca_seq_table.v, 0, 4096u, 0x00020000);
  unsigned char* const my_flags = smem + OFF_FLAG + wid * 16;
  const unsigned flag_addr0 = (unsigned)(size_t)(__attribute__((address_space(3))) unsigned char*)my_flags;
  if (lane < 4) {
    asm volatile("ds_write_b32 %0, %1\n\ts_waitcnt lgkmcnt(0)" ::"v"(flag_addr0 + (unsigned)lane * 4u), "v"(0xFFFFFFFFu) : "memory");
  }

  int d_c = my_lane, d_k = 0, d_s = 0;
  int d_n = 0;
  unsigned d_v1[2], d_v2[2];
  auto head_slab = [&]() {
    int lane_o = lane;
// ... 89 lines not shown
      u32x4 fb[TN];
#pragma unroll
      for (int j = 0; j < TN; ++j) {
        __builtin_amdgcn_sched_barrier(0);
        fb[j] = *reinterpret_cast<const u32x4*>(wb + j * 16 * WLD_B + kq * 64);
      }
      __builtin_amdgcn_sched_barrier(0);
#define CA_WRES_PAIR(J, CNT)                                        \
  asm volatile("s_waitcnt lgkmcnt(" #CNT ")" ::: "memory");         \
  __builtin_amdgcn_sched_barrier(0);                                \
  acc[0][J] = Elem<DT>::mfma(fb[J], fa0, acc[0][J]);                \
  acc[1][J] = Elem<DT>::mfma(fb[J], fa1, acc[1][J]);                \
  __builtin_amdgcn_sched_barrier(0);
      CA_WRES_PAIR(0, 9)
      if (p.ln_inline) {
#pragma unroll
        for (int q = 0; q < 4; ++q) {
          const float a0 = Elem<DT>::to_f((u16)(fa0[q] & 0xffffu)), a1 = Elem<DT>::to_f((u16)(fa0[q] >> 16));
          const float b0 = Elem<DT>::to_f((u16)(fa1[q] & 0xffffu)), b1 = Elem<DT>::to_f((u16)(fa1[q] >> 16));
          ln_s[0] += a0 + a1;
          ln_ss[0] = fmaf(a0, a0, fmaf(a1, a1, ln_ss[0]));
          ln_s[1] += b0 + b1;
          ln_ss[1] = fmaf(b0, b0, fmaf(b1, b1, ln_ss[1]));
        }
      }
      CA_WRES_PAIR(1, 8) CA_WRES_PAIR(2, 7) CA_WRES_PAIR(3, 6) CA_WRES_PAIR(4, 5)
      unsigned flag_next;
      asm volatile("ds_read_b32 %0, %1" : "=v"(flag_next) : "v"(flag_addr0 + (unsigned)((r_n + 1) % 3) * 4u) : "memory");
      __builtin_amdgcn_sched_barrier(0);
      CA_WRES_PAIR(5, 5) CA_WRES_PAIR(6, 4) CA_WRES_PAIR(7, 3) CA_WRES_PAIR(8, 2) CA_WRES_PAIR(9, 1)
#undef CA_WRES_PAIR
      asm volatile("s_waitcnt lgkmcnt(0)" : "+v"(flag_next)::"memory");
      r_s = r_s == 2 ? 0 : r_s + 1;
      ++r_n;
      chunk_wait(r_n, flag_next);
    }

    if (p.ln_inline) {
#pragma unroll
      for (int i = 0; i < 2; ++i) {
        float a = ln_s[i], b = ln_ss[i];
        a += __shfl_xor(a, 16);
        b += __shfl_xor(b, 16);
        a += __shfl_xor(a, 32);
        b += __shfl_xor(b, 32);
        const float mean = a * (1.f / K);
        st[i] = make_float2(mean, rsqrtf(fmaxf(b * (1.f / K) - mean * mean, 0.f) + p.ln_eps));
      }
    }
    if (p.dbg == 1) {
      if (acc[0][0][0] == 12345.678f) *reinterpret_cast<float*>(p.c) = acc[1][TN - 1][1];
      continue;
    }
    int lane_e = lane;
    asm volatile("" : "+v"(lane_e));
    const int g = lane_e >> 4, l15 = lane_e & 15;
    u32x4 rr[2][TN / 2];
    if (p.res) {
#pragma unroll
      for (int i = 0; i < 2; ++i)
#pragma unroll
        for (int q = 0; q < TN / 2; ++q) {
          const int m = m0 + i * 16 + l15;
          const unsigned off = m < p.m ? ((unsigned)m * (unsigned)p.ld_res + (unsigned)(n0 + g * 8)) * 2u : 0x80000000u;
          rr[i][q] = __builtin_bit_cast(u32x4, __builtin_amdgcn_raw_buffer_load_b128(rs_res, off, q * 64, 0));
        }
    }
    if (p.alpha == 1.f && p.post == 1.f && p.act == CA_ACT_NONE && !p.geglu) {
      unsigned off[2];
#pragma unroll
      for (int i = 0; i < 2; ++i) {
        const int m = m0 + i * 16 + l15;
        off[i] = m < p.m ? ((unsigned)m * (unsigned)p.ldc + (unsigned)(n0 + g * 8)) * 2u : 0x80000000u;
      }
#pragma unroll
      for (int q = 0; q < TN / 2; ++q) {
        f32x4 bb[2], cs[2];
#pragma unroll
        for (int u = 0; u < 2; ++u) {
          const int col = 32 * q + 8 * g + 4 * u;
          bb[u] = *reinterpret_cast<const f32x4*>(smem + OFF_PAR + col * 4);
          cs[u] = (f32x4){0.f, 0.f, 0.f, 0.f};
          if (p.ln_colsum) cs[u] = *reinterpret_cast<const f32x4*>(smem + OFF_PAR + (PN + col) * 4);
          if (p.rowbias) {
            const f32x4 rb = *reinterpret_cast<const f32x4*>(rb_patch + col * 4);
#pragma unroll
            for (int r = 0; r < 4; ++r) bb[u][r] += rb[r];
          }
        }
#pragma unroll
        for (int i = 0; i < 2; ++i) {
          u32x4 w;
#pragma unroll
          for (int u = 0; u < 2; ++u) {
            f32x4 v = acc[i][2 * q + u];
            if (p.ln_colsum) {
#pragma unroll
              for (int r = 0; r < 4; ++r) v[r] = st[i].y * (v[r] - st[i].x * cs[u][r]);
            }
            w[2 * u] = pack2<DT>(v[0] + bb[u][0], v[1] + bb[u][1]);
            w[2 * u + 1] = pack2<DT>(v[2] + bb[u][2], v[3] + bb[u][3]);
          }
          if (p.res) {
#pragma unroll
            for (int k = 0; k < 4; ++k) {
              if (DT == CA_F16) {
                unsigned s_;
                asm("v_pk_add_f16 %0, %1, %2" : "=v"(s_) : "v"(w[k]), "v"(rr[i][q][k]));
                w[k] = s_;
              } else {
                w[k] = pack2<DT>(Elem<DT>::to_f((u16)(w[k] & 0xffffu)) + Elem<DT>::to_f((u16)(rr[i][q][k] & 0xffffu)),
                                 Elem<DT>::to_f((u16)(w[k] >> 16)) + Elem<DT>::to_f((u16)(rr[i][q][k] >> 16)));
              }
            }
          }
          __builtin_amdgcn_raw_buffer_store_b128(w, rs_c, off[i] + (unsigned)(q * 64), 0, 0);
        }
      }
      continue;
    }
    if (p.geglu && !p.rowbias && !p.res && p.alpha == 1.f && p.post == 1.f && p.act == CA_ACT_NONE) {
      unsigned off[2];
#pragma unroll
      for (int i = 0; i < 2; ++i) {
        const int m = m0 + i * 16 + l15;
        off[i] = m < p.m ? ((unsigned)m * (unsigned)p.ldc + (unsigned)((n0 >> 1) + g * 2)) * 2u : DMA_OOB;
      }
#pragma unroll
      for (int j = 0; j < TN; ++j) {
        const f32x4 bi = *reinterpret_cast<const f32x4*>(smem + OFF_PAR + (j * 16 + g * 4) * 4);
        f32x4 cs = {0.f, 0.f, 0.f, 0.f};
        if (p.ln_colsum) cs = *reinterpret_cast<const f32x4*>(smem + OFF_PAR + (PN + j * 16 + g * 4) * 4);
#pragma unroll
        for (int i = 0; i < 2; ++i) {
          f32x4 v = acc[i][j];
          if (p.ln_colsum) {
#pragma unroll
            for (int r = 0; r < 4; ++r) v[r] = st[i].y * (v[r] - st[i].x * cs[r]);
          }
          float h[4];
#pragma unroll
          for (int r = 0; r < 4; ++r) h[r] = Elem<DT>::to_f(Elem<DT>::from_f(v[r] + bi[r]));
          const f32x2 gg = gelu_erf_f2((f32x2){h[1], h[3]});
          __builtin_amdgcn_raw_buffer_store_b32(pack2<DT>(h[0] * gg[0], h[2] * gg[1]), rs_c, off[i], j * 16, 0);
        }
      }
      continue;
    }
#pragma unroll
    for (int j = 0; j < TN; ++j) {
      const int nl = ca_wres_col(j, 4 * g, geglu);
      const f32x4 bi = *reinterpret_cast<const f32x4*>(smem + OFF_PAR + nl * 4);
      f32x4 cs = {0.f, 0.f, 0.f, 0.f}, rb = {0.f, 0.f, 0.f, 0.f};
      if (p.ln_colsum) cs = *reinterpret_cast<const f32x4*>(smem + OFF_PAR + (PN + nl) * 4);
      if (p.rowbias) rb = *reinterpret_cast<const f32x4*>(rb_patch + nl * 4);
#pragma unroll
      for (int i = 0; i < 2; ++i) {
        const int m = m0 + i * 16 + l15;
        float v[4];
#pragma unroll
        for (int r = 0; r < 4; ++r) v[r] = acc[i][j][r];
        if (p.ln_colsum) {
#pragma unroll
          for (int r = 0; r < 4; ++r) v[r] = st[i].y * (v[r] - st[i].x * cs[r]);
        }
#pragma unroll
        for (int r = 0; r < 4; ++r) v[r] = Elem<DT>::to_f(Elem<DT>::from_f((v[r] + bi[r] + rb[r]) * p.alpha));
        if (p.res) {
          const unsigned r0 = rr[i][j >> 1][2 * (j & 1)], r1 = rr[i][j >> 1][2 * (j & 1) + 1];
          v[0] += Elem<DT>::to_f((u16)(r0 & 0xffffu));
          v[1] += Elem<DT>::to_f((u16)(r0 >> 16));
          v[2] += Elem<DT>::to_f((u16)(r1 & 0xffffu));
          v[3] += Elem<DT>::to_f((u16)(r1 >> 16));
        }
#pragma unroll
        for (int r = 0; r < 4; ++r) v[r] *= p.post;
        if (p.act != CA_ACT_NONE) {
#pragma unroll
          for (int r = 0; r < 4; ++r) v[r] = act_f(v[r], p.act);
        }
        if (p.geglu) {
          const f32x2 gg = gelu_erf_f2((f32x2){v[1], v[3]});
          const unsigned w = pack2<DT>(v[0] * gg[0], v[2] * gg[1]);
          const unsigned off = m < p.m ? ((unsigned)m * (unsigned)p.ldc + (unsigned)((n0 >> 1) + (nl >> 1))) * 2u : 0x80000000u;
          __builtin_amdgcn_raw_buffer_store_b32(w, rs_c, off, 0, 0);
        } else {
          u32x2 w;
          w[0] = pack2<DT>(v[0], v[1]);
          w[1] = pack2<DT>(v[2], v[3]);
          const unsigned off = m < p.m ? ((unsigned)m * (unsigned)p.ldc + (unsigned)(n0 + nl)) * 2u : 0x80000000u;
          __builtin_amdgcn_raw_buffer_store_b64(w, rs_c, off, 0, 0);
        }
      }
    }
    asm volatile("s_waitcnt lgkmcnt(0)" ::: "memory");
  }
  asm volatile("s_waitcnt vmcnt(0)" ::: "memory");
}
```

### controlanimate_amd/kernels.py

```python
from __future__ import annotations

import ctypes as C
from typing import Optional

import torch

from . import _capi
from .context import dispatch
from ._capi import (AttnArgs, ConvArgs, ConvNarrowArgs, FfArgs, PerceiverAttnArgs, TattnArgs, XattnArgs, GemmArgs, GroupNormArgs, LayerNormArgs, CA_ACT_NONE,
                    CA_ACT_SILU, CA_BF16, CA_F16, check, lib)

ACT_NONE, ACT_SILU = CA_ACT_NONE, CA_ACT_SILU
ACT_QUICK_GELU, ACT_GELU = 2, 3
ACT_RELU = _capi.CA_ACT_RELU
ACT_RELU6 = _capi.CA_ACT_RELU6


def dt_code(dtype: torch.dtype) -> int:
    if dtype == torch.bfloat16:
        return CA_BF16
    if dtype == torch.float16:
        return CA_F16
    raise TypeError(f"activations must be bf16 or fp16, got {dtype}")


def _stream() -> int:
    return torch.cuda.current_stream().cuda_stream


def _p(t: Optional[torch.Tensor]) -> Optional[int]:
    return None if t is None else t.data_ptr()


def _req_cuda(*ts):
    for t in ts:
        if t is not None and not t.is_cuda:
            raise _capi.CAHipError("HIP kernels need device tensors (no CPU fallback)")


_plan_sink = None


def _record_plan(query, args) -> None:
    if _plan_sink is not None:
        buf = C.create_string_buffer(64)
        _plan_sink.append(buf.value.decode() if query(C.byref(args), buf, 64) == 0 else "?")


def gemm(a: torch.Tensor, w: torch.Tensor, *, a2: Optional[torch.Tensor] = None,
         bias: Optional[torch.Tensor] = None, rowbias: Optional[torch.Tensor] = None,
         rows_per_group: int = 0, residual: Optional[torch.Tensor] = None, alpha: float = 1.0,
         post_scale: float = 1.0, act: int = ACT_NONE, geglu: bool = False, out_f32: bool = False,
         out: Optional[torch.Tensor] = None, ln=None, row_sums: bool = False) -> torch.Tensor:
    _req_cuda(a, w, a2, bias, rowbias, residual, out)
    assert a.dim() == 2 and a.stride(1) == 1 and w.dim() == 2 and w.is_contiguous()
    m, k1 = a.shape
    k2 = 0
    if a2 is not None:
        assert a2.dim() == 2 and a2.stride(1) == 1 and a2.shape[0] == m and a2.dtype == a.dtype
        k2 = a2.shape[1]
    n = w.shape[0]
    assert w.shape[1] == k1 + k2 and w.dtype == a.dtype
    ncols = n // 2 if geglu else n
    if out is None:
        out = torch.empty((m, ncols), device=a.device, dtype=torch.float32 if out_f32 else a.dtype)
    assert out.shape == (m, ncols) and out.stride(1) == 1
    if residual is not None:
        assert residual.shape == (m, n) and residual.stride(1) == 1 and residual.dtype == a.dtype
    if bias is not None:
        assert bias.dtype == torch.float32 and bias.numel() == n
    if rowbias is not None:
        assert rowbias.dtype == torch.float32 and rowbias.dim() == 2 and rowbias.shape[1] == n and rows_per_group > 0
    args = GemmArgs(a=_p(a), a2=_p(a2), w=_p(w), c=_p(out), bias=_p(bias), rowbias=_p(rowbias),
                    residual=_p(residual), lda=a.stride(0), lda2=a2.stride(0) if a2 is not None else 0,
                    ldc=out.stride(0), ld_res=residual.stride(0) if residual is not None else 0,
                    ld_rowbias=rowbias.stride(0) if rowbias is not None else 0,
                    m=m, n=n, k1=k1, k2=k2, rows_per_group=rows_per_group, alpha=alpha,
                    post_scale=post_scale, act=act, geglu=int(geglu), out_f32=int(out_f32),
                    dtype=dt_code(a.dtype))
    frag = getattr(w, "_frag", None)
    if frag is not None and frag[1] == bool(geglu) and dispatch.gemm_ar:
        args.w_frag = _p(frag[0])
    if ln is not None:
        st, cs = ln
        assert cs.dtype == torch.float32 and cs.numel() == n
        args.ln_colsum = _p(cs)
        if isinstance(st, RowStats):
            assert st.x.data_ptr() == a.data_ptr() and st.x.shape == a.shape, "RowStats belongs to another tensor"
            args.ln_eps = st.eps
            if lib().ca_gemm_ln_inline_supported(C.byref(args)):
                pass
            elif st.sums is not None:
                rs, parts = st.sums
                assert rs.shape == (m, parts, 2) and rs.dtype == torch.float32 and rs.is_contiguous()
                args.ln_stats, args.ln_parts = _p(rs), min(parts, 4)
                if parts > 4 or lib().ca_gemm_wants_finished_stats(C.byref(args)):
                    fin = getattr(st, "_finished", None)
                    if fin is None:
                        fin = torch.empty((m, 2), device=a.device, dtype=torch.float32)
                        check(lib().ca_ln_finish_sums(_p(rs), parts, m, k1 + k2, st.eps, _p(fin), _stream()), "ca_ln_finish_sums")
                        st._finished = fin
                    args.ln_stats, args.ln_parts = _p(fin), 0
            else:
                st = st.tensor()
        if not isinstance(st, RowStats):
            assert st.dtype == torch.float32 and st.shape == (m, 2) and st.is_contiguous()
            args.ln_stats = _p(st)
    if hasattr(out, "_row_sums"):
        del out._row_sums
    if row_sums and dispatch.ln_row_sums and not geglu and not out_f32:
        parts = int(lib().ca_gemm_row_sums_parts(C.byref(args)))
        if parts > 0:
            rs = torch.empty((m, parts, 2), device=a.device, dtype=torch.float32)
            args.row_sums_out = _p(rs)
            out._row_sums = (rs, parts)
    wbytes = 0 if args.row_sums_out else int(lib().ca_gemm_workspace_bytes(C.byref(args)))
    if wbytes > 0:
        ws = torch.empty((wbytes,), device=a.device, dtype=torch.uint8)
        args.workspace, args.workspace_bytes = _p(ws), wbytes
    _record_plan(lib().ca_gemm_plan_name, args)
    check(lib().ca_gemm(C.byref(args), _stream()), "ca_gemm")
    return out


def attach_w_frag(w: torch.Tensor, geglu: bool = False) -> torch.Tensor:
    _req_cuda(w)
    if w.dim() != 2 or w.shape[1] != 320 or w.shape[0] % 320 != 0 or not w.is_contiguous() or w.dtype not in (torch.float16, torch.bfloat16):
        return w
    dst = torch.empty_like(w)
    check(lib().ca_pack_w_frag(w.data_ptr(), w.shape[0], w.shape[1], int(bool(geglu)), dst.data_ptr(), _stream()), "ca_pack_w_frag")
    w._frag = (dst, bool(geglu))
    return w


def ff_fused(x: torch.Tensor, w1_frag: torch.Tensor, bias1: torch.Tensor, colsum1: torch.Tensor, w2_frag: torch.Tensor,
             bias2: Optional[torch.Tensor], ln_eps: float, residual: Optional[torch.Tensor] = None,
             ln_stats: Optional[torch.Tensor] = None, *, w_out_frag: Optional[torch.Tensor] = None, bias_out: Optional[torch.Tensor] = None,
             residual_out: Optional[torch.Tensor] = None) -> Optional[torch.Tensor]:
    if not dispatch.ff_fused:
        return None
    _req_cuda(x, w1_frag, bias1, colsum1, w2_frag, bias2, residual, ln_stats, w_out_frag, bias_out, residual_out)
    if x.dim() != 2 or x.stride(1) != 1 or (residual is not None and (residual.shape != x.shape or residual.stride(1) != 1 or residual.dtype != x.dtype)):
        return None
    if w_out_frag is None and (bias_out is not None or residual_out is not None):
        return None
    if residual_out is not None and (residual_out.shape != x.shape or residual_out.stride(1) != 1 or residual_out.dtype != x.dtype):
        return None
    m, c = x.shape
    inner = w2_frag.shape[1]
    y = torch.empty((m, c), device=x.device, dtype=x.dtype)
    args = FfArgs(x=_p(x), w1_frag=_p(w1_frag), bias1=_p(bias1), colsum1=_p(colsum1), ln_stats=_p(ln_stats), w2_frag=_p(w2_frag),
                  bias2=_p(bias2), residual=_p(residual), y=_p(y), lda=x.stride(0), ldc=y.stride(0),
                  ld_res=residual.stride(0) if residual is not None else 0, m=m, c=c, inner=inner, ln_eps=float(ln_eps), dtype=dt_code(x.dtype),
                  w_out_frag=_p(w_out_frag), bias_out=_p(bias_out), residual_out=_p(residual_out),
                  ld_res_out=residual_out.stride(0) if residual_out is not None else 0)
    if not lib().ca_ff_fused_supported(C.byref(args)):
        return None
    if _plan_sink is not None:
        _plan_sink.append("ff_out128" if w_out_frag is not None else "ff_fused128")
    check(lib().ca_ff_fused(C.byref(args), _stream()), "ca_ff_fused")
    return y


def tattn_fused(x: torch.Tensor, w_frag: torch.Tensor, gamma: torch.Tensor, bias_pe: torch.Tensor, b: int, frames: int, tokens: int,
                heads: int, ln_eps: float, scale: float, *, w_out_frag: Optional[torch.Tensor] = None, bias_out: Optional[torch.Tensor] = None,
                residual: Optional[torch.Tensor] = None) -> Optional[torch.Tensor]:
    if not dispatch.tattn_fused:
        return None
    _req_cuda(x, w_frag, gamma, bias_pe, w_out_frag, bias_out, residual)
    if x.dim() != 2 or x.stride(1) != 1 or x.shape[0] != b * frames * tokens or bias_pe.shape[0] < frames or bias_pe.stride(1) != 1:
        return None
    if w_out_frag is None and (bias_out is not None or residual is not None):
        return None
    if residual is not None and (residual.shape != x.shape or residual.stride(1) != 1 or residual.dtype != x.dtype):
        return None
    c = x.shape[1]
    o = torch.empty((x.shape[0], c), device=x.device, dtype=x.dtype)
# ... 1658 lines not shown
```

### include/controlanimate_hip.h

```cpp
#ifndef CONTROLANIMATE_HIP_H
#define CONTROLANIMATE_HIP_H

#include <stdint.h>

#ifdef __cplusplus
extern "C" {
#endif

#define CA_ABI_VERSION 16

#define CA_BF16 0
#define CA_F16 1
#define CA_F32 2

#define CA_OK 0
#define CA_ERR_INVALID_ARG (-1)
#define CA_ERR_UNSUPPORTED (-2)
#define CA_ERR_LAUNCH (-3)

#define CA_ACT_NONE 0
#define CA_ACT_SILU 1
#define CA_ACT_QUICK_GELU 2
#define CA_ACT_GELU 3
#define CA_ACT_RELU 4
#define CA_ACT_RELU6 5
#define CA_ACT_LEAKY02 6

int ca_abi_version(void);
const char* ca_last_error(void);

typedef struct ca_gemm_args {
  const void* a;
  const void* a2;
  const void* w;
  void* c;
  const float* bias;
  const float* rowbias;
  const void* residual;
  int64_t lda, lda2, ldc, ld_res, ld_rowbias;
  int32_t m, n, k1, k2;
  int32_t rows_per_group;
  float alpha, post_scale;
  int32_t act;
  int32_t geglu;
  int32_t out_f32;
  int32_t dtype;
  const float* ln_stats;
  const float* ln_colsum;
  float ln_eps;
  void* workspace;
  int64_t workspace_bytes;
  float* row_sums_out;
  int32_t ln_parts;
  const void* w_frag;
} ca_gemm_args;
int ca_gemm(const ca_gemm_args* args, void* stream);
int ca_pack_w_frag(const void* w, int32_t n, int32_t k, int32_t geglu, void* dst, void* stream);
typedef struct ca_ff_args {
  const void* x;
  const void* w1_frag;
  const float* bias1;
  const float* colsum1;
  const float* ln_stats;
  const void* w2_frag;
  const float* bias2;
  const void* residual;
  void* y;
  int64_t lda, ldc, ld_res;
  int32_t m, c, inner;
  float ln_eps;
  int32_t dtype;
  const void* w_out_frag;
  const float* bias_out;
  const void* residual_out;
  int64_t ld_res_out;
} ca_ff_args;
int ca_ff_fused(const ca_ff_args* args, void* stream);
int ca_ff_fused_supported(const ca_ff_args* args);
int ca_pack_w2_frag(const void* w, int32_t n, int32_t k, void* dst, void* stream);
#define CA_TATTN_W_FRAG_ELEMS 368640
typedef struct ca_tattn_args {
  const void* x;
  const void* w_frag;
  const float* gamma;
  const float* bias_pe;
  void* o;
  int64_t lda, ldo, ld_bias_pe;
  int32_t batch, frames, tokens, heads, c;
  float ln_eps, scale;
  int32_t dtype;
  const void* w_out_frag;
  const float* bias_out;
  const void* residual;
  int64_t ld_res;
} ca_tattn_args;
int ca_tattn_fused(const ca_tattn_args* args, void* stream);
int ca_tattn_fused_supported(const ca_tattn_args* args);
#define CA_ATTN_WOUT_FRAG_ELEMS 102400
int ca_pack_w_out(const void* w, int32_t n, int32_t k, void* dst, void* stream);
int ca_pack_w_tattn(const void* w, int32_t n, int32_t k, void* dst, void* stream);
#define CA_XATTN_W_FRAG_ELEMS 122880
#define CA_XATTN_KV_FRAG_ELEMS 7680
typedef struct ca_xattn_args {
  const void* x;
  const void* wq_frag;
  const float* bias;
  const void* kv_frag;
  void* o;
  int64_t lda, ldo;
// ... 455 lines not shown
```

Baseline: 15.88.

## Compute ControlNet zero-conv GEMM once and write both CFG copies in epilogue

When a zero-conv output has to be duplicated for the two classifier-free-guidance halves, the GEMM now runs once with an out_reps=2 option. The epilogue loops over the copies and applies a per-copy residual offset, replacing two full GEMM launches over the same input. This adds out_reps plumbing through the C ABI, the plan validation and several kernel epilogues (DMA, WRES, PS/PP2). It also adds a support probe that falls back to the per-copy launches, at the cost of a longer epilogue and extra template instances.

```diff
diff --git a/controlanimate_amd/_capi.py b/controlanimate_amd/_capi.py
--- a/controlanimate_amd/_capi.py
+++ b/controlanimate_amd/_capi.py
@@ -46,6 +46,7 @@
         ("workspace", C.c_void_p), ("workspace_bytes", C.c_int64),
         ("row_sums_out", C.c_void_p), ("ln_parts", C.c_int32),
         ("w_frag", C.c_void_p),
+        ("c_rep_stride", C.c_int64), ("res_rep_stride", C.c_int64), ("out_reps", C.c_int32),
     ]
 
 
@@ -201,6 +202,7 @@
     "ca_xattn_pack_w": (C.c_int, [C.c_void_p, C.c_int32, C.c_int32, C.c_void_p, C.c_void_p]),
     "ca_xattn_pack_kv": (C.c_int, [C.c_void_p, C.c_int64, C.c_int32, C.c_int32, C.c_int32, C.c_int32, C.c_float, C.c_int32, C.c_void_p, C.c_void_p]),
     "ca_gemm_ln_inline_supported": (C.c_int, [C.POINTER(GemmArgs)]),
+    "ca_gemm_out_reps_supported": (C.c_int, [C.POINTER(GemmArgs)]),
     "ca_gemm_wants_finished_stats": (C.c_int, [C.POINTER(GemmArgs)]),
     "ca_ln_finish_sums": (C.c_int, [C.c_void_p, C.c_int, C.c_int64, C.c_int, C.c_float, C.c_void_p, C.c_void_p]),
     "ca_gemm_workspace_bytes": (C.c_int64, [C.POINTER(GemmArgs)]),
diff --git a/controlanimate_amd/context.py b/controlanimate_amd/context.py
--- a/controlanimate_amd/context.py
+++ b/controlanimate_amd/context.py
@@ -42,6 +42,7 @@
     ln_fold = True
     cfg_shared = True
     cn_cfg_dedup = True
+    zero_conv_once = True
     pdc_block_fused = True
     dpt_head_fused = False
     pose_conv7_direct = True
diff --git a/controlanimate_amd/controlnet.py b/controlanimate_amd/controlnet.py
--- a/controlanimate_amd/controlnet.py
+++ b/controlanimate_amd/controlnet.py
@@ -212,6 +212,7 @@
 
     @torch.no_grad()
     def apply_zero_convs(self, outs, x, scales, accumulate: Optional[Tuple[List[torch.Tensor], torch.Tensor]] = None, twice: bool = False):
+        from .context import dispatch
         def one(zc, o, scale, prev):
             B_, h, w, c = o.shape
             rows = B_ * h * w
@@ -219,6 +220,10 @@
             if not twice:
                 return zc.run(a, alpha=scale, residual=None if prev is None else prev.view(rows, c)).view(B_, h, w, c)
             full = torch.empty((2 * B_, h, w, c), device=o.device, dtype=o.dtype)
+            res = None if prev is None else prev.view(2 * rows, c)
+            if dispatch.zero_conv_once and K.gemm_out_reps_supported(a, zc.w.t, bias=zc.b.t, residual=res, alpha=scale, out_reps=2):
+                zc.run(a, alpha=scale, residual=res, out=full.view(2 * rows, c), out_reps=2)
+                return full
             for hf in range(2):
                 zc.run(a, alpha=scale, residual=None if prev is None else prev.view(2 * rows, c)[hf * rows:(hf + 1) * rows],
                        out=full.view(2 * rows, c)[hf * rows:(hf + 1) * rows])
diff --git a/controlanimate_amd/csrc/ca_gemm.hip b/controlanimate_amd/csrc/ca_gemm.hip
--- a/controlanimate_amd/csrc/ca_gemm.hip
+++ b/controlanimate_amd/csrc/ca_gemm.hip
@@ -140,7 +140,7 @@
 }
 
 
-template <int DT, int BM, int BN, int WAVES_M, int WAVES_N, int MODE, int NBUF>
+template <int DT, int BM, int BN, int WAVES_M, int WAVES_N, int MODE, int NBUF, bool REPS = false>
 __global__ __launch_bounds__(256, NBUF == 1 ? (BN > 128 ? 3 : 4) : 2)
 void k_gemm_dma(GemmKParams p) {
   static_assert(WAVES_M * WAVES_N == 4 && (NBUF == 1 || NBUF == 3), "instantiations: see above");
@@ -325,7 +325,7 @@
     }
     return;
   }
-  gemm_epilogue<DT, BM, BN, TM, TN, NT>(p, acc, smem, m0, n0, wm, wn, l15, g, tid);
+  gemm_epilogue<DT, BM, BN, TM, TN, NT, false, REPS>(p, acc, smem, m0, n0, wm, wn, l15, g, tid);
 }
 
 template <int DT>
@@ -407,6 +407,15 @@
       hipLaunchKernelGGL((k_splitk_reduce<DT>), dim3(ceil_div_i((int64_t)p.m * (p.n / 8), 256)), dim3(256), 0, st, p);
       return CA_OK;
     case PK_DMA:
+      if (p.out_reps > 1) {
+        if (MODE != 0) break;
+        if (g.bn == 160 && g.nbuf == 1) hipLaunchKernelGGL((k_gemm_dma<DT, 128, 160, 2, 2, 0, 1, true>), grid, dim3(256), 0, st, p);
+        else if (g.bn == 128 && g.nbuf == 1) hipLaunchKernelGGL((k_gemm_dma<DT, 128, 128, 2, 2, 0, 1, true>), grid, dim3(256), 0, st, p);
+        else if (g.bn == 64 && g.nbuf == 1) hipLaunchKernelGGL((k_gemm_dma<DT, 128, 64, 4, 1, 0, 1, true>), grid, dim3(256), 0, st, p);
+        else if (g.bn == 64 && g.nbuf == 3) hipLaunchKernelGGL((k_gemm_dma<DT, 128, 64, 4, 1, 0, 3, true>), grid, dim3(256), 0, st, p);
+        else break;
+        return CA_OK;
+      }
       if (g.bn == 160 && g.nbuf == 1) hipLaunchKernelGGL((k_gemm_dma<DT, 128, 160, 2, 2, MODE, 1>), grid, dim3(256), 0, st, p);
       else if (g.bn == 128 && g.nbuf == 1) hipLaunchKernelGGL((k_gemm_dma<DT, 128, 128, 2, 2, MODE, 1>), grid, dim3(256), 0, st, p);
       else if (g.bn == 64 && g.nbuf == 1) hipLaunchKernelGGL((k_gemm_dma<DT, 128, 64, 4, 1, MODE, 1>), grid, dim3(256), 0, st, p);
@@ -445,6 +454,11 @@
   DenseAsk ask{};
   ask.without_row_sums = true;
   return gemm_resolve(a, d, ask) == CA_OK ? row_sums_parts_of(d.p) : 0;
+}
+
+extern "C" int ca_gemm_out_reps_supported(const ca_gemm_args* a) {
+  DenseLaunch d;
+  return a && a->out_reps > 1 && gemm_prepare(a, d) == CA_OK ? 1 : 0;
 }
 
 extern "C" int ca_gemm_ln_inline_supported(const ca_gemm_args* a) {
diff --git a/controlanimate_amd/csrc/ca_gemm_core.h b/controlanimate_amd/csrc/ca_gemm_core.h
--- a/controlanimate_amd/csrc/ca_gemm_core.h
+++ b/controlanimate_amd/csrc/ca_gemm_core.h
@@ -38,6 +38,8 @@
   unsigned w_group_stride;
   int up2_rows, up2_tiles;
   unsigned up2_mag_w, up2_mag_h;
+  int out_reps;
+  int64_t c_rep_stride, res_rep_stride;
 };
 
 constexpr int BK = 64;
@@ -136,7 +138,7 @@
   }
 }
 
-template <int DT, int BM, int BN, int TM, int TN, int NT = 256, bool ROWSUM = false>
+template <int DT, int BM, int BN, int TM, int TN, int NT = 256, bool ROWSUM = false, bool REPS = false>
 __device__ __forceinline__ void gemm_epilogue(const GemmKParams& p, f32x4 (&acc)[TM][TN], u16* cs, int m0, int n0, int wm, int wn,
                                               int l15, int g, int tid, float2* rs = nullptr) {
   if (p.n < 8) {
@@ -231,96 +233,39 @@
   constexpr int CH = BN / 8;
   const bool simple = p.post == 1.f && p.act == CA_ACT_NONE && !p.geglu && !p.out_f32;
   const bool geglu_only = p.geglu && p.post == 1.f && p.act == CA_ACT_NONE && !p.res && !p.out_f32;
-#pragma unroll
-  for (int u = 0; u < BM * CH / NT; ++u) {
-    const int id = tid + u * NT;
-    const int row = id / CH, c8 = id - row * CH;
-    const int m = m0 + row, n = n0 + c8 * 8;
-    if (m >= p.m || n >= p.n) continue;
-    if (simple) {
-      u32x4 pk = ld16(cs + row * CLD + c8 * 8);
-      if (p.res) {
-        const u32x4 rr = ld16(p.res + (int64_t)m * p.ld_res + n);
-        if (DT == CA_F16) {
-#pragma unroll
-          for (int k = 0; k < 4; ++k) {
-            unsigned s_;
-            asm("v_pk_add_f16 %0, %1, %2" : "=v"(s_) : "v"(pk[k]), "v"(rr[k]));
-            pk[k] = s_;
+  const int reps = REPS ? p.out_reps : 1;
+  for (int rep = 0; rep < reps; ++rep) {
+    const u16* const res_r = REPS && p.res ? p.res + (int64_t)rep * p.res_rep_stride : p.res;
+    void* const c_r = REPS ? (void*)(reinterpret_cast<u16*>(p.c) + (int64_t)rep * p.c_rep_stride) : p.c;
+    int tid_r = tid;
+    if (REPS) asm volatile("" : "+v"(tid_r));
+#pragma unroll
+    for (int u = 0; u < BM * CH / NT; ++u) {
+      const int id = tid_r + u * NT;
+      const int row = id / CH, c8 = id - row * CH;
+      const int m = m0 + row, n = n0 + c8 * 8;
+      if (m >= p.m || n >= p.n) continue;
+      if (simple) {
+        u32x4 pk = ld16(cs + row * CLD + c8 * 8);
+        if (res_r) {
+          const u32x4 rr = ld16(res_r + (int64_t)m * p.ld_res + n);
+          if (DT == CA_F16) {
+#pragma unroll
+            for (int k = 0; k < 4; ++k) {
+              unsigned s_;
+              asm("v_pk_add_f16 %0, %1, %2" : "=v"(s_) : "v"(pk[k]), "v"(rr[k]));
+              pk[k] = s_;
+            }
+          } else {
+            float a_[8], r_[8];
+            unpack8<DT>(pk, a_);
+            unpack8<DT>(rr, r_);
+#pragma unroll
+            for (int k = 0; k < 8; ++k) a_[k] += r_[k];
+            pk = pack8<DT>(a_);
           }
-        } else {
-          float a_[8], r_[8];
-          unpack8<DT>(pk, a_);
-          unpack8<DT>(rr, r_);
-#pragma unroll
-          for (int k = 0; k < 8; ++k) a_[k] += r_[k];
-          pk = pack8<DT>(a_);
-        }
-      }
-      st16(reinterpret_cast<u16*>(p.c) + (int64_t)m * p.ldc + n, pk);
-      if (ROWSUM && p.row_sums) {
-        float r[8];
-        unpack8<DT>(pk, r);
-        float a = 0.f, b = 0.f;
-#pragma unroll
-        for (int k = 0; k < 8; ++k) {
-          a += r[k];
-          b = fmaf(r[k], r[k], b);
-        }
-        rs[row * CH + c8] = make_float2(a, b);
-      }
-      continue;
-    }
-    if (geglu_only) {
-      float v[8];
-      unpack8<DT>(ld16(cs + row * CLD + c8 * 8), v);
-      const f32x2 g0 = gelu_erf_f2((f32x2){v[1], v[3]}), g1 = gelu_erf_f2((f32x2){v[5], v[7]});
-      u32x2 w;
-      w[0] = pack2<DT>(v[0] * g0[0], v[2] * g0[1]);
-      w[1] = pack2<DT>(v[4] * g1[0], v[6] * g1[1]);
-      *reinterpret_cast<u32x2*>(reinterpret_cast<u16*>(p.c) + (int64_t)m * p.ldc + (n >> 1)) = w;
-      continue;
-    }
-    float v[8];
-    unpack8<DT>(ld16(cs + row * CLD + c8 * 8), v);
-    if (p.res) {
-      float r[8];
-      unpack8<DT>(ld16(p.res + (int64_t)m * p.ld_res + n), r);
-#pragma unroll
-      for (int k = 0; k < 8; ++k) v[k] += r[k];
-    }
-#pragma unroll
-    for (int k = 0; k < 8; ++k) v[k] *= p.post;
-    if (p.act != CA_ACT_NONE) {
-#pragma unroll
-      for (int k = 0; k < 8; ++k) v[k] = act_f(v[k], p.act);
-    }
-    if (p.geglu) {
-      float o[4];
-#pragma unroll
-      for (int k = 0; k < 4; k += 2) {
-        const f32x2 gg = gelu_erf_f2((f32x2){v[2 * k + 1], v[2 * k + 3]});
-        o[k] = v[2 * k] * gg[0];
-        o[k + 1] = v[2 * k + 2] * gg[1];
-      }
-      const int64_t off = (int64_t)m * p.ldc + (n >> 1);
-      if (p.out_f32) {
-        *reinterpret_cast<f32x4*>(reinterpret_cast<float*>(p.c) + off) = (f32x4){o[0], o[1], o[2], o[3]};
-      } else {
-        u32x2 w;
-        w[0] = pack2<DT>(o[0], o[1]);
-        w[1] = pack2<DT>(o[2], o[3]);
-        *reinterpret_cast<u32x2*>(reinterpret_cast<u16*>(p.c) + off) = w;
-      }
-    } else {
-      const int64_t off = (int64_t)m * p.ldc + n;
-      if (p.out_f32) {
-        float* cp = reinterpret_cast<float*>(p.c) + off;
-        *reinterpret_cast<f32x4*>(cp) = (f32x4){v[0], v[1], v[2], v[3]};
-        *reinterpret_cast<f32x4*>(cp + 4) = (f32x4){v[4], v[5], v[6], v[7]};
-      } else {
-        const u32x4 pk = pack8<DT>(v);
-        st16(reinterpret_cast<u16*>(p.c) + off, pk);
+        }
+        st16(reinterpret_cast<u16*>(c_r) + (int64_t)m * p.ldc + n, pk);
         if (ROWSUM && p.row_sums) {
           float r[8];
           unpack8<DT>(pk, r);
@@ -331,6 +276,70 @@
             b = fmaf(r[k], r[k], b);
           }
           rs[row * CH + c8] = make_float2(a, b);
+        }
+        continue;
+      }
+      if (geglu_only) {
+        float v[8];
+        unpack8<DT>(ld16(cs + row * CLD + c8 * 8), v);
+        const f32x2 g0 = gelu_erf_f2((f32x2){v[1], v[3]}), g1 = gelu_erf_f2((f32x2){v[5], v[7]});
+        u32x2 w;
+        w[0] = pack2<DT>(v[0] * g0[0], v[2] * g0[1]);
+        w[1] = pack2<DT>(v[4] * g1[0], v[6] * g1[1]);
+        *reinterpret_cast<u32x2*>(reinterpret_cast<u16*>(c_r) + (int64_t)m * p.ldc + (n >> 1)) = w;
+        continue;
+      }
+      float v[8];
+      unpack8<DT>(ld16(cs + row * CLD + c8 * 8), v);
+      if (res_r) {
+        float r[8];
+        unpack8<DT>(ld16(res_r + (int64_t)m * p.ld_res + n), r);
+#pragma unroll
+        for (int k = 0; k < 8; ++k) v[k] += r[k];
+      }
+#pragma unroll
+      for (int k = 0; k < 8; ++k) v[k] *= p.post;
+      if (p.act != CA_ACT_NONE) {
+#pragma unroll
+        for (int k = 0; k < 8; ++k) v[k] = act_f(v[k], p.act);
+      }
+      if (p.geglu) {
+        float o[4];
+#pragma unroll
+        for (int k = 0; k < 4; k += 2) {
+          const f32x2 gg = gelu_erf_f2((f32x2){v[2 * k + 1], v[2 * k + 3]});
+          o[k] = v[2 * k] * gg[0];
+          o[k + 1] = v[2 * k + 2] * gg[1];
+        }
+        const int64_t off = (int64_t)m * p.ldc + (n >> 1);
+        if (p.out_f32) {
+          *reinterpret_cast<f32x4*>(reinterpret_cast<float*>(c_r) + off) = (f32x4){o[0], o[1], o[2], o[3]};
+        } else {
+          u32x2 w;
+          w[0] = pack2<DT>(o[0], o[1]);
+          w[1] = pack2<DT>(o[2], o[3]);
+          *reinterpret_cast<u32x2*>(reinterpret_cast<u16*>(c_r) + off) = w;
+        }
+      } else {
+        const int64_t off = (int64_t)m * p.ldc + n;
+        if (p.out_f32) {
+          float* cp = reinterpret_cast<float*>(c_r) + off;
+          *reinterpret_cast<f32x4*>(cp) = (f32x4){v[0], v[1], v[2], v[3]};
+          *reinterpret_cast<f32x4*>(cp + 4) = (f32x4){v[4], v[5], v[6], v[7]};
+        } else {
+          const u32x4 pk = pack8<DT>(v);
+          st16(reinterpret_cast<u16*>(c_r) + off, pk);
+          if (ROWSUM && p.row_sums) {
+            float r[8];
+            unpack8<DT>(pk, r);
+            float a = 0.f, b = 0.f;
+#pragma unroll
+            for (int k = 0; k < 8; ++k) {
+              a += r[k];
+              b = fmaf(r[k], r[k], b);
+            }
+            rs[row * CH + c8] = make_float2(a, b);
+          }
         }
       }
     }
@@ -368,6 +377,9 @@
 inline int64_t out_rows(const GemmKParams& p) { return p.up2_rows ? 4 * (int64_t)p.up2_rows : (int64_t)p.m; }
 inline int64_t c_extent_bytes(const GemmKParams& p) { return ((out_rows(p) - 1) * p.ldc + (p.geglu ? p.n / 2 : p.n)) * 2; }
 inline int64_t res_extent_bytes(const GemmKParams& p) { return p.res ? ((out_rows(p) - 1) * p.ld_res + p.n) * 2 : 0; }
+inline int64_t rep_span(const GemmKParams& p, int64_t stride) { return p.out_reps > 1 ? (int64_t)(p.out_reps - 1) * stride * 2 : 0; }
+inline unsigned c_desc_bytes(const GemmKParams& p) { return (unsigned)(c_extent_bytes(p) + rep_span(p, p.c_rep_stride)); }
+inline unsigned res_desc_bytes(const GemmKParams& p) { return p.res ? (unsigned)(res_extent_bytes(p) + rep_span(p, p.res_rep_stride)) : 0u; }
 inline bool act_out_fit31(const GemmKParams& p) {
   return c_extent_bytes(p) < FIT31 && res_extent_bytes(p) < FIT31 && p.a_bytes < FIT31 && (!p.c2 || p.a2_bytes < FIT31);
 }
diff --git a/controlanimate_amd/csrc/ca_gemm_plan.h b/controlanimate_amd/csrc/ca_gemm_plan.h
--- a/controlanimate_amd/csrc/ca_gemm_plan.h
+++ b/controlanimate_amd/csrc/ca_gemm_plan.h
@@ -202,6 +202,22 @@
   p.rows_per_group = a->rows_per_group > 0 ? a->rows_per_group : 1;
   p.alpha = a->alpha, p.post = a->post_scale, p.act = a->act, p.geglu = a->geglu, p.out_f32 = a->out_f32;
   p.splits = 1;
+  CA_REQUIRE(a->out_reps >= 0, "ca_gemm: out_reps=%d", a->out_reps);
+  if (a->out_reps > 1) {
+    CA_REQUIRE(!a->geglu && !a->ln_colsum && !a->ln_stats && !a->row_sums_out && !a->out_f32 && a->n >= 8,
+               "ca_gemm: out_reps is not implemented with GEGLU, a folded LayerNorm, row_sums_out, fp32 output or N < 8");
+    const int64_t c_ext = (int64_t)(a->m - 1) * a->ldc + a->n, res_ext = a->residual ? (int64_t)(a->m - 1) * a->ld_res + a->n : 0;
+    CA_REQUIRE(a->c_rep_stride % 8 == 0 && a->c_rep_stride >= c_ext, "ca_gemm: c_rep_stride=%lld must be a multiple of 8 and at least one copy's extent "
+               "(%lld elements): the copies must not overlap", (long long)a->c_rep_stride, (long long)c_ext);
+    CA_REQUIRE(!a->residual || (a->res_rep_stride % 8 == 0 && a->res_rep_stride >= 0), "ca_gemm: res_rep_stride=%lld must be a multiple of 8 and >= 0",
+               (long long)a->res_rep_stride);
+    const int64_t lim = FIT31 / 2;
+    CA_REQUIRE(a->ldc >= 0 && a->c_rep_stride < lim && c_ext < lim && (int64_t)(a->out_reps - 1) * a->c_rep_stride + c_ext < lim,
+               "ca_gemm: the %d copies of the output must end below 2^31 bytes", a->out_reps);
+    CA_REQUIRE(!a->residual || (a->ld_res >= 0 && a->res_rep_stride < lim && res_ext < lim && (int64_t)(a->out_reps - 1) * a->res_rep_stride + res_ext < lim),
+               "ca_gemm: the %d copies of the residual must end below 2^31 bytes", a->out_reps);
+    p.out_reps = a->out_reps, p.c_rep_stride = a->c_rep_stride, p.res_rep_stride = a->residual ? a->res_rep_stride : 0;
+  }
   return CA_OK;
 }
 
@@ -232,6 +248,10 @@
   CA_REQUIRE(!d.p.row_sums || row_sums_capable(d.p), "ca_gemm: row_sums_out is not available for this launch: ask ca_gemm_row_sums_parts() first");
   CA_REQUIRE(!d.p.ln_inline || wres_eligible(d.p), "ca_gemm: in-kernel LayerNorm statistics (ln_stats NULL) are not available for this launch: "
              "ask ca_gemm_ln_inline_supported() first and pass ln_stats otherwise");
+  const PlanKind k = d.plan.kind;
+  CA_REQUIRE(d.p.out_reps <= 1 || k == PK_WRES || k == PK_PS || k == PK_PP2 || k == PK_DMA,
+             "ca_gemm: out_reps is not implemented by the kernel this launch gets (split-K, the 256 x 320, activation-resident and register-staged "
+             "kernels): ask ca_gemm_out_reps_supported() first and issue one launch per copy otherwise");
   return CA_OK;
 }
 
diff --git a/controlanimate_amd/csrc/ca_gemm_pp.hip b/controlanimate_amd/csrc/ca_gemm_pp.hip
--- a/controlanimate_amd/csrc/ca_gemm_pp.hip
+++ b/controlanimate_amd/csrc/ca_gemm_pp.hip
@@ -49,7 +49,9 @@
 
 template <int DT, int MODE>
 int launch_pp(const GemmKParams& p, PlanKind kind, unsigned tiles, hipStream_t st) {
-  const unsigned c_bytes = (unsigned)c_extent_bytes(p), res_bytes = (unsigned)res_extent_bytes(p);
+  const unsigned c_bytes = c_desc_bytes(p), res_bytes = res_desc_bytes(p);
+  const bool reps = p.out_reps > 1;
+  if (reps && (MODE != 0 || kind == PK_PQ)) return CA_ERR_LAUNCH;
   const unsigned grid = tiles < (unsigned)cu_count() ? tiles : (unsigned)cu_count();
   switch (kind) {
     case PK_PQ: {
@@ -65,7 +67,10 @@
       return CA_OK;
     }
     case PK_PS: {
-      auto launch = [&](const GemmKParams& q) { hipLaunchKernelGGL((k_gemm_ps<DT, MODE>), dim3(grid), dim3(512), 0, st, q, (int)tiles, c_bytes, res_bytes); };
+      auto launch = [&](const GemmKParams& q) {
+        if (reps) hipLaunchKernelGGL((k_gemm_ps<DT, 0, true>), dim3(grid), dim3(512), 0, st, q, (int)tiles, c_bytes, res_bytes);
+        else hipLaunchKernelGGL((k_gemm_ps<DT, MODE>), dim3(grid), dim3(512), 0, st, q, (int)tiles, c_bytes, res_bytes);
+      };
 #ifdef CA_STAMPS
       if (p.dbg == 9) return launch_stamped(p, st, "ps", 8, 10, launch);
 #endif
@@ -80,11 +85,14 @@
       if (per * 8 > chunks) per = chunks / 8;
       if (per < 1) per = 1;
       const unsigned rb_bytes = p.rowbias ? (unsigned)(((int64_t)((p.m - 1) / p.rows_per_group) * p.ld_rowbias + p.n) * 4) : 16u;
-      hipLaunchKernelGGL((k_gemm_wres<DT>), dim3(8 * per * panels), dim3(512), 0, st, p, panels, 8 * per, chunks, rb_bytes, c_bytes, res_bytes);
+      if (reps) hipLaunchKernelGGL((k_gemm_wres<DT, true>), dim3(8 * per * panels), dim3(512), 0, st, p, panels, 8 * per, chunks, rb_bytes, c_bytes, res_bytes);
+      else hipLaunchKernelGGL((k_gemm_wres<DT>), dim3(8 * per * panels), dim3(512), 0, st, p, panels, 8 * per, chunks, rb_bytes, c_bytes, res_bytes);
       return CA_OK;
     }
     case PK_PP2:
-      hipLaunchKernelGGL((k_gemm_pp2<DT, MODE>), dim3(tiles), dim3(512), 0, st, p);
+      if (reps && p.splits > 1) return CA_ERR_LAUNCH;
+      if (reps) hipLaunchKernelGGL((k_gemm_pp2<DT, 0, true>), dim3(tiles), dim3(512), 0, st, p);
+      else hipLaunchKernelGGL((k_gemm_pp2<DT, MODE>), dim3(tiles), dim3(512), 0, st, p);
       return CA_OK;
     default: return CA_ERR_LAUNCH;
   }
diff --git a/controlanimate_amd/csrc/ca_gemm_pp2.h b/controlanimate_amd/csrc/ca_gemm_pp2.h
--- a/controlanimate_amd/csrc/ca_gemm_pp2.h
+++ b/controlanimate_amd/csrc/ca_gemm_pp2.h
@@ -1,4 +1,4 @@
-template <int DT, int MODE>
+template <int DT, int MODE, bool REPS = false>
 __global__ __launch_bounds__(512, 2) void k_gemm_pp2(GemmKParams p) {
   constexpr int BM = 128, BN = 320, KT = 64;
   constexpr int TM = 4, TN = 5;
@@ -223,5 +223,5 @@
     }
     return;
   }
-  gemm_epilogue<DT, BM, BN, TM, TN, 512, true>(p, acc, smem, m0, n0, wr, wc, l15, g, tid, reinterpret_cast<float2*>(smem + BM * (BN + 8)));
+  gemm_epilogue<DT, BM, BN, TM, TN, 512, true, REPS>(p, acc, smem, m0, n0, wr, wc, l15, g, tid, reinterpret_cast<float2*>(smem + BM * (BN + 8)));
 }
diff --git a/controlanimate_amd/csrc/ca_gemm_ps.h b/controlanimate_amd/csrc/ca_gemm_ps.h
--- a/controlanimate_amd/csrc/ca_gemm_ps.h
+++ b/controlanimate_amd/csrc/ca_gemm_ps.h
@@ -45,7 +45,7 @@
   return 32 * (j >> 1) + 8 * (i >> 2) + 4 * (j & 1) + (i & 3);
 }
 
-template <int DT, int MODE>
+template <int DT, int MODE, bool REPS = false>
 __global__ __launch_bounds__(512, 2) void k_gemm_ps(GemmKParams p, int tiles_total, unsigned c_bytes, unsigned res_bytes) {
   constexpr int BM = 128, BN = 320, KT = 64;
   constexpr int TM = 4, TN = 5;
@@ -303,14 +303,14 @@
     res8[i] = (u32x2){0u, 0u};
   }
   int mark_res = 0;
-  auto res_prefetch = [&](int m0, int n0) __attribute__((always_inline)) {
+  auto res_prefetch = [&](int m0, int n0, unsigned sh = 0u) __attribute__((always_inline)) {
     int lane_o = lane;
     asm volatile("" : "+v"(lane_o));
     const int l15o = lane_o & 15, go = lane_o >> 4;
 #pragma unroll
     for (int i = 0; i < TM; ++i) {
       const int m = m0 + wr * 64 + i * 16 + l15o;
-      const unsigned rowoff = m < p.m ? (unsigned)m * (unsigned)p.ld_res * 2u + (unsigned)(n0 + wc * 80) * 2u : OOB_V;
+      const unsigned rowoff = m < p.m ? (unsigned)m * (unsigned)p.ld_res * 2u + (unsigned)(n0 + wc * 80) * 2u + sh : OOB_V;
       const unsigned o0 = rowoff + (unsigned)(8 * go) * 2u, o1 = rowoff + (unsigned)(32 + 8 * go) * 2u, o2 = rowoff + (unsigned)(64 + 4 * go) * 2u;
       asm volatile("s_nop 4\n\tbuffer_load_dwordx4 %0, %3, %6, 0 offen\n\tbuffer_load_dwordx4 %1, %4, %6, 0 offen\n\tbuffer_load_dwordx2 %2, %5, %6, 0 offen"
                    : "=&v"(res16[i][0]), "=&v"(res16[i][1]), "=&v"(res8[i])
@@ -437,60 +437,69 @@
       q.rb = *reinterpret_cast<const f32x4*>(rbp + c0 * 4);
       return q;
     };
-    auto staged = [&](int i, int j, const Par& q, float (&v)[4]) __attribute__((always_inline)) {
+    auto staged = [&](int i, int j, const Par& q, float (&v)[4], bool clear = true) __attribute__((always_inline)) {
 #pragma unroll
       for (int r = 0; r < 4; ++r) {
         float x = st[i].y * (acc[i][j][r] - st[i].x * q.cs[r]);
         x = (x + q.bi[r]) + q.rb[r];
         v[r] = x * p.alpha;
       }
-      acc[i][j] = (f32x4){0.f, 0.f, 0.f, 0.f};
+      if (clear) acc[i][j] = (f32x4){0.f, 0.f, 0.f, 0.f};
     };
 
     if (p.res) res_wait();
     if (!geglu) {
-#pragma unroll
-      for (int pr = 0; pr < 3; ++pr) {
-        const int nq = pr < 2 ? 2 : 1;
-        Par par[2];
-#pragma unroll
-        for (int u = 0; u < 2; ++u)
-          if (u < nq) par[u] = load_par(wc * 80 + (pr < 2 ? 32 * pr + 8 * g + 4 * u : 64 + 4 * g));
-#pragma unroll
-        for (int i = 0; i < TM; ++i) {
-          unsigned w[4] = {0u, 0u, 0u, 0u};
-#pragma unroll
-          for (int u = 0; u < 2; ++u) {
-            if (u >= nq) break;
-            float v[4];
-            staged(i, pr * 2 + u, par[u], v);
-            w[2 * u] = pack2<DT>(v[0], v[1]);
-            w[2 * u + 1] = pack2<DT>(v[2], v[3]);
-          }
-#pragma unroll
-          for (int k = 0; k < 4; ++k) {
-            if (k >= 2 * nq) break;
-            const unsigned rr = pr < 2 ? res16[i][pr & 1][k] : res8[i][k & 1];
-            if (DT == CA_F16) {
-              unsigned s_;
-              asm("v_pk_add_f16 %0, %1, %2" : "=v"(s_) : "v"(w[k]), "v"(rr));
-              w[k] = s_;
-            } else {
-              w[k] = pack2<DT>(Elem<DT>::to_f((u16)(w[k] & 0xffffu)) + Elem<DT>::to_f((u16)(rr & 0xffffu)),
-                               Elem<DT>::to_f((u16)(w[k] >> 16)) + Elem<DT>::to_f((u16)(rr >> 16)));
+      const int reps = REPS ? p.out_reps : 1;
+      for (int rep = 0; rep < reps; ++rep) {
+        const bool last = !REPS || rep + 1 == reps;
+        const unsigned c_sh = REPS ? (unsigned)rep * (unsigned)p.c_rep_stride * 2u : 0u;
+        if (REPS && rep > 0 && p.res) {
+          res_prefetch(m0, n0, (unsigned)rep * (unsigned)p.res_rep_stride * 2u);
+          res_wait();
+        }
+#pragma unroll
+        for (int pr = 0; pr < 3; ++pr) {
+          const int nq = pr < 2 ? 2 : 1;
+          Par par[2];
+#pragma unroll
+          for (int u = 0; u < 2; ++u)
+            if (u < nq) par[u] = load_par(wc * 80 + (pr < 2 ? 32 * pr + 8 * g + 4 * u : 64 + 4 * g));
+#pragma unroll
+          for (int i = 0; i < TM; ++i) {
+            unsigned w[4] = {0u, 0u, 0u, 0u};
+#pragma unroll
+            for (int u = 0; u < 2; ++u) {
+              if (u >= nq) break;
+              float v[4];
+              staged(i, pr * 2 + u, par[u], v, last);
+              w[2 * u] = pack2<DT>(v[0], v[1]);
+              w[2 * u + 1] = pack2<DT>(v[2], v[3]);
             }
-          }
-          if (p.row_sums) {
 #pragma unroll
             for (int k = 0; k < 4; ++k) {
               if (k >= 2 * nq) break;
-              const float lo = Elem<DT>::to_f((u16)(w[k] & 0xffffu)), hi = Elem<DT>::to_f((u16)(w[k] >> 16));
-              rsum[i] += lo + hi;
-              rsq[i] = fmaf(lo, lo, fmaf(hi, hi, rsq[i]));
+              const unsigned rr = pr < 2 ? res16[i][pr & 1][k] : res8[i][k & 1];
+              if (DT == CA_F16) {
+                unsigned s_;
+                asm("v_pk_add_f16 %0, %1, %2" : "=v"(s_) : "v"(w[k]), "v"(rr));
+                w[k] = s_;
+              } else {
+                w[k] = pack2<DT>(Elem<DT>::to_f((u16)(w[k] & 0xffffu)) + Elem<DT>::to_f((u16)(rr & 0xffffu)),
+                                 Elem<DT>::to_f((u16)(w[k] >> 16)) + Elem<DT>::to_f((u16)(rr >> 16)));
+              }
             }
+            if (p.row_sums) {
+#pragma unroll
+              for (int k = 0; k < 4; ++k) {
+                if (k >= 2 * nq) break;
+                const float lo = Elem<DT>::to_f((u16)(w[k] & 0xffffu)), hi = Elem<DT>::to_f((u16)(w[k] >> 16));
+                rsum[i] += lo + hi;
+                rsq[i] = fmaf(lo, lo, fmaf(hi, hi, rsq[i]));
+              }
+            }
+            if (pr < 2) __builtin_amdgcn_raw_buffer_store_b128((u32x4){w[0], w[1], w[2], w[3]}, rs_c, rowoff[i] + c_sh + (unsigned)(32 * pr + 8 * g) * 2u, 0, 0);
+            else __builtin_amdgcn_raw_buffer_store_b64((u32x2){w[0], w[1]}, rs_c, rowoff[i] + c_sh + (unsigned)(64 + 4 * g) * 2u, 0, 0);
           }
-          if (pr < 2) __builtin_amdgcn_raw_buffer_store_b128((u32x4){w[0], w[1], w[2], w[3]}, rs_c, rowoff[i] + (unsigned)(32 * pr + 8 * g) * 2u, 0, 0);
-          else __builtin_amdgcn_raw_buffer_store_b64((u32x2){w[0], w[1]}, rs_c, rowoff[i] + (unsigned)(64 + 4 * g) * 2u, 0, 0);
         }
       }
       issued += 3 * TM;
diff --git a/controlanimate_amd/csrc/ca_gemm_wres.h b/controlanimate_amd/csrc/ca_gemm_wres.h
--- a/controlanimate_amd/csrc/ca_gemm_wres.h
+++ b/controlanimate_amd/csrc/ca_gemm_wres.h
@@ -5,7 +5,7 @@
   return 32 * (j >> 1) + 8 * (i >> 2) + 4 * (j & 1) + (i & 3);
 }
 
-template <int DT>
+template <int DT, bool REPS = false>
 __global__ __launch_bounds__(512, 1) void k_gemm_wres(GemmKParams p, int panels, int lanes, int chunks, unsigned rb_bytes, unsigned c_bytes, unsigned res_bytes) {
   constexpr int K = 320, PN = 160, TN = 10, KQ = 10;
   constexpr int WLD_B = 656;
@@ -201,148 +201,152 @@
       if (acc[0][0][0] == 12345.678f) *reinterpret_cast<float*>(p.c) = acc[1][TN - 1][1];
       continue;
     }
-    int lane_e = lane;
-    asm volatile("" : "+v"(lane_e));
-    const int g = lane_e >> 4, l15 = lane_e & 15;
-    u32x4 rr[2][TN / 2];
-    if (p.res) {
-#pragma unroll
-      for (int i = 0; i < 2; ++i)
+    const int reps = REPS ? p.out_reps : 1;
+    for (int rep = 0; rep < reps; ++rep) {
+      const unsigned c_sh = REPS ? (unsigned)rep * (unsigned)p.c_rep_stride * 2u : 0u, res_sh = REPS ? (unsigned)rep * (unsigned)p.res_rep_stride * 2u : 0u;
+      int lane_e = lane;
+      asm volatile("" : "+v"(lane_e));
+      const int g = lane_e >> 4, l15 = lane_e & 15;
+      u32x4 rr[2][TN / 2];
+      if (p.res) {
+#pragma unroll
+        for (int i = 0; i < 2; ++i)
+#pragma unroll
+          for (int q = 0; q < TN / 2; ++q) {
+            const int m = m0 + i * 16 + l15;
+            const unsigned off = m < p.m ? ((unsigned)m * (unsigned)p.ld_res + (unsigned)(n0 + g * 8)) * 2u + res_sh : 0x80000000u;
+            rr[i][q] = __builtin_bit_cast(u32x4, __builtin_amdgcn_raw_buffer_load_b128(rs_res, off, q * 64, 0));
+          }
+      }
+      if (p.alpha == 1.f && p.post == 1.f && p.act == CA_ACT_NONE && !p.geglu) {
+        unsigned off[2];
+#pragma unroll
+        for (int i = 0; i < 2; ++i) {
+          const int m = m0 + i * 16 + l15;
+          off[i] = m < p.m ? ((unsigned)m * (unsigned)p.ldc + (unsigned)(n0 + g * 8)) * 2u + c_sh : 0x80000000u;
+        }
 #pragma unroll
         for (int q = 0; q < TN / 2; ++q) {
-          const int m = m0 + i * 16 + l15;
-          const unsigned off = m < p.m ? ((unsigned)m * (unsigned)p.ld_res + (unsigned)(n0 + g * 8)) * 2u : 0x80000000u;
-          rr[i][q] = __builtin_bit_cast(u32x4, __builtin_amdgcn_raw_buffer_load_b128(rs_res, off, q * 64, 0));
-        }
-    }
-    if (p.alpha == 1.f && p.post == 1.f && p.act == CA_ACT_NONE && !p.geglu) {
-      unsigned off[2];
-#pragma unroll
-      for (int i = 0; i < 2; ++i) {
-        const int m = m0 + i * 16 + l15;
-        off[i] = m < p.m ? ((unsigned)m * (unsigned)p.ldc + (unsigned)(n0 + g * 8)) * 2u : 0x80000000u;
-      }
-#pragma unroll
-      for (int q = 0; q < TN / 2; ++q) {
-        f32x4 bb[2], cs[2];
-#pragma unroll
-        for (int u = 0; u < 2; ++u) {
-          const int col = 32 * q + 8 * g + 4 * u;
-          bb[u] = *reinterpret_cast<const f32x4*>(smem + OFF_PAR + col * 4);
-          cs[u] = (f32x4){0.f, 0.f, 0.f, 0.f};
-          if (p.ln_colsum) cs[u] = *reinterpret_cast<const f32x4*>(smem + OFF_PAR + (PN + col) * 4);
-          if (p.rowbias) {
-            const f32x4 rb = *reinterpret_cast<const f32x4*>(rb_patch + col * 4);
-#pragma unroll
-            for (int r = 0; r < 4; ++r) bb[u][r] += rb[r];
-          }
-        }
-#pragma unroll
-        for (int i = 0; i < 2; ++i) {
-          u32x4 w;
+          f32x4 bb[2], cs[2];
 #pragma unroll
           for (int u = 0; u < 2; ++u) {
-            f32x4 v = acc[i][2 * q + u];
-            if (p.ln_colsum) {
-#pragma unroll
-              for (int r = 0; r < 4; ++r) v[r] = st[i].y * (v[r] - st[i].x * cs[u][r]);
+            const int col = 32 * q + 8 * g + 4 * u;
+            bb[u] = *reinterpret_cast<const f32x4*>(smem + OFF_PAR + col * 4);
+            cs[u] = (f32x4){0.f, 0.f, 0.f, 0.f};
+            if (p.ln_colsum) cs[u] = *reinterpret_cast<const f32x4*>(smem + OFF_PAR + (PN + col) * 4);
+            if (p.rowbias) {
+              const f32x4 rb = *reinterpret_cast<const f32x4*>(rb_patch + col * 4);
+#pragma unroll
+              for (int r = 0; r < 4; ++r) bb[u][r] += rb[r];
             }
-            w[2 * u] = pack2<DT>(v[0] + bb[u][0], v[1] + bb[u][1]);
-            w[2 * u + 1] = pack2<DT>(v[2] + bb[u][2], v[3] + bb[u][3]);
-          }
-          if (p.res) {
-#pragma unroll
-            for (int k = 0; k < 4; ++k) {
-              if (DT == CA_F16) {
-                unsigned s_;
-                asm("v_pk_add_f16 %0, %1, %2" : "=v"(s_) : "v"(w[k]), "v"(rr[i][q][k]));
-                w[k] = s_;
-              } else {
-                w[k] = pack2<DT>(Elem<DT>::to_f((u16)(w[k] & 0xffffu)) + Elem<DT>::to_f((u16)(rr[i][q][k] & 0xffffu)),
-                                 Elem<DT>::to_f((u16)(w[k] >> 16)) + Elem<DT>::to_f((u16)(rr[i][q][k] >> 16)));
+          }
+#pragma unroll
+          for (int i = 0; i < 2; ++i) {
+            u32x4 w;
+#pragma unroll
+            for (int u = 0; u < 2; ++u) {
+              f32x4 v = acc[i][2 * q + u];
+              if (p.ln_colsum) {
+#pragma unroll
+                for (int r = 0; r < 4; ++r) v[r] = st[i].y * (v[r] - st[i].x * cs[u][r]);
+              }
+              w[2 * u] = pack2<DT>(v[0] + bb[u][0], v[1] + bb[u][1]);
+              w[2 * u + 1] = pack2<DT>(v[2] + bb[u][2], v[3] + bb[u][3]);
+            }
+            if (p.res) {
+#pragma unroll
+              for (int k = 0; k < 4; ++k) {
+                if (DT == CA_F16) {
+                  unsigned s_;
+                  asm("v_pk_add_f16 %0, %1, %2" : "=v"(s_) : "v"(w[k]), "v"(rr[i][q][k]));
+                  w[k] = s_;
+                } else {
+                  w[k] = pack2<DT>(Elem<DT>::to_f((u16)(w[k] & 0xffffu)) + Elem<DT>::to_f((u16)(rr[i][q][k] & 0xffffu)),
+                                   Elem<DT>::to_f((u16)(w[k] >> 16)) + Elem<DT>::to_f((u16)(rr[i][q][k] >> 16)));
+                }
               }
             }
-          }
-          __builtin_amdgcn_raw_buffer_store_b128(w, rs_c, off[i] + (unsigned)(q * 64), 0, 0);
-        }
-      }
-      continue;
-    }
-    if (p.geglu && !p.rowbias && !p.res && p.alpha == 1.f && p.post == 1.f && p.act == CA_ACT_NONE) {
-      unsigned off[2];
-#pragma unroll
-      for (int i = 0; i < 2; ++i) {
-        const int m = m0 + i * 16 + l15;
-        off[i] = m < p.m ? ((unsigned)m * (unsigned)p.ldc + (unsigned)((n0 >> 1) + g * 2)) * 2u : DMA_OOB;
+            __builtin_amdgcn_raw_buffer_store_b128(w, rs_c, off[i] + (unsigned)(q * 64), 0, 0);
+          }
+        }
+        continue;
+      }
+      if (p.geglu && !p.rowbias && !p.res && p.alpha == 1.f && p.post == 1.f && p.act == CA_ACT_NONE) {
+        unsigned off[2];
+#pragma unroll
+        for (int i = 0; i < 2; ++i) {
+          const int m = m0 + i * 16 + l15;
+          off[i] = m < p.m ? ((unsigned)m * (unsigned)p.ldc + (unsigned)((n0 >> 1) + g * 2)) * 2u + c_sh : DMA_OOB;
+        }
+#pragma unroll
+        for (int j = 0; j < TN; ++j) {
+          const f32x4 bi = *reinterpret_cast<const f32x4*>(smem + OFF_PAR + (j * 16 + g * 4) * 4);
+          f32x4 cs = {0.f, 0.f, 0.f, 0.f};
+          if (p.ln_colsum) cs = *reinterpret_cast<const f32x4*>(smem + OFF_PAR + (PN + j * 16 + g * 4) * 4);
+#pragma unroll
+          for (int i = 0; i < 2; ++i) {
+            f32x4 v = acc[i][j];
+            if (p.ln_colsum) {
+#pragma unroll
+              for (int r = 0; r < 4; ++r) v[r] = st[i].y * (v[r] - st[i].x * cs[r]);
+            }
+            float h[4];
+#pragma unroll
+            for (int r = 0; r < 4; ++r) h[r] = Elem<DT>::to_f(Elem<DT>::from_f(v[r] + bi[r]));
+            const f32x2 gg = gelu_erf_f2((f32x2){h[1], h[3]});
+            __builtin_amdgcn_raw_buffer_store_b32(pack2<DT>(h[0] * gg[0], h[2] * gg[1]), rs_c, off[i], j * 16, 0);
+          }
+        }
+        continue;
       }
 #pragma unroll
       for (int j = 0; j < TN; ++j) {
-        const f32x4 bi = *reinterpret_cast<const f32x4*>(smem + OFF_PAR + (j * 16 + g * 4) * 4);
-        f32x4 cs = {0.f, 0.f, 0.f, 0.f};
-        if (p.ln_colsum) cs = *reinterpret_cast<const f32x4*>(smem + OFF_PAR + (PN + j * 16 + g * 4) * 4);
+        const int nl = ca_wres_col(j, 4 * g, geglu);
+        const f32x4 bi = *reinterpret_cast<const f32x4*>(smem + OFF_PAR + nl * 4);
+        f32x4 cs = {0.f, 0.f, 0.f, 0.f}, rb = {0.f, 0.f, 0.f, 0.f};
+        if (p.ln_colsum) cs = *reinterpret_cast<const f32x4*>(smem + OFF_PAR + (PN + nl) * 4);
+        if (p.rowbias) rb = *reinterpret_cast<const f32x4*>(rb_patch + nl * 4);
 #pragma unroll
         for (int i = 0; i < 2; ++i) {
-          f32x4 v = acc[i][j];
+          const int m = m0 + i * 16 + l15;
+          float v[4];
+#pragma unroll
+          for (int r = 0; r < 4; ++r) v[r] = acc[i][j][r];
           if (p.ln_colsum) {
 #pragma unroll
             for (int r = 0; r < 4; ++r) v[r] = st[i].y * (v[r] - st[i].x * cs[r]);
           }
-          float h[4];
-#pragma unroll
-          for (int r = 0; r < 4; ++r) h[r] = Elem<DT>::to_f(Elem<DT>::from_f(v[r] + bi[r]));
-          const f32x2 gg = gelu_erf_f2((f32x2){h[1], h[3]});
-          __builtin_amdgcn_raw_buffer_store_b32(pack2<DT>(h[0] * gg[0], h[2] * gg[1]), rs_c, off[i], j * 16, 0);
-        }
-      }
-      continue;
-    }
-#pragma unroll
-    for (int j = 0; j < TN; ++j) {
-      const int nl = ca_wres_col(j, 4 * g, geglu);
-      const f32x4 bi = *reinterpret_cast<const f32x4*>(smem + OFF_PAR + nl * 4);
-      f32x4 cs = {0.f, 0.f, 0.f, 0.f}, rb = {0.f, 0.f, 0.f, 0.f};
-      if (p.ln_colsum) cs = *reinterpret_cast<const f32x4*>(smem + OFF_PAR + (PN + nl) * 4);
-      if (p.rowbias) rb = *reinterpret_cast<const f32x4*>(rb_patch + nl * 4);
-#pragma unroll
-      for (int i = 0; i < 2; ++i) {
-        const int m = m0 + i * 16 + l15;
-        float v[4];
-#pragma unroll
-        for (int r = 0; r < 4; ++r) v[r] = acc[i][j][r];
-        if (p.ln_colsum) {
-#pragma unroll
-          for (int r = 0; r < 4; ++r) v[r] = st[i].y * (v[r] - st[i].x * cs[r]);
-        }
-#pragma unroll
-        for (int r = 0; r < 4; ++r) v[r] = Elem<DT>::to_f(Elem<DT>::from_f((v[r] + bi[r] + rb[r]) * p.alpha));
-        if (p.res) {
-          const unsigned r0 = rr[i][j >> 1][2 * (j & 1)], r1 = rr[i][j >> 1][2 * (j & 1) + 1];
-          v[0] += Elem<DT>::to_f((u16)(r0 & 0xffffu));
-          v[1] += Elem<DT>::to_f((u16)(r0 >> 16));
-          v[2] += Elem<DT>::to_f((u16)(r1 & 0xffffu));
-          v[3] += Elem<DT>::to_f((u16)(r1 >> 16));
-        }
-#pragma unroll
-        for (int r = 0; r < 4; ++r) v[r] *= p.post;
-        if (p.act != CA_ACT_NONE) {
-#pragma unroll
-          for (int r = 0; r < 4; ++r) v[r] = act_f(v[r], p.act);
-        }
-        if (p.geglu) {
-          const f32x2 gg = gelu_erf_f2((f32x2){v[1], v[3]});
-          const unsigned w = pack2<DT>(v[0] * gg[0], v[2] * gg[1]);
-          const unsigned off = m < p.m ? ((unsigned)m * (unsigned)p.ldc + (unsigned)((n0 >> 1) + (nl >> 1))) * 2u : 0x80000000u;
-          __builtin_amdgcn_raw_buffer_store_b32(w, rs_c, off, 0, 0);
-        } else {
-          u32x2 w;
-          w[0] = pack2<DT>(v[0], v[1]);
-          w[1] = pack2<DT>(v[2], v[3]);
-          const unsigned off = m < p.m ? ((unsigned)m * (unsigned)p.ldc + (unsigned)(n0 + nl)) * 2u : 0x80000000u;
-          __builtin_amdgcn_raw_buffer_store_b64(w, rs_c, off, 0, 0);
-        }
-      }
-    }
-    asm volatile("s_waitcnt lgkmcnt(0)" ::: "memory");
+#pragma unroll
+          for (int r = 0; r < 4; ++r) v[r] = Elem<DT>::to_f(Elem<DT>::from_f((v[r] + bi[r] + rb[r]) * p.alpha));
+          if (p.res) {
+            const unsigned r0 = rr[i][j >> 1][2 * (j & 1)], r1 = rr[i][j >> 1][2 * (j & 1) + 1];
+            v[0] += Elem<DT>::to_f((u16)(r0 & 0xffffu));
+            v[1] += Elem<DT>::to_f((u16)(r0 >> 16));
+            v[2] += Elem<DT>::to_f((u16)(r1 & 0xffffu));
+            v[3] += Elem<DT>::to_f((u16)(r1 >> 16));
+          }
+#pragma unroll
+          for (int r = 0; r < 4; ++r) v[r] *= p.post;
+          if (p.act != CA_ACT_NONE) {
+#pragma unroll
+            for (int r = 0; r < 4; ++r) v[r] = act_f(v[r], p.act);
+          }
+          if (p.geglu) {
+            const f32x2 gg = gelu_erf_f2((f32x2){v[1], v[3]});
+            const unsigned w = pack2<DT>(v[0] * gg[0], v[2] * gg[1]);
+            const unsigned off = m < p.m ? ((unsigned)m * (unsigned)p.ldc + (unsigned)((n0 >> 1) + (nl >> 1))) * 2u + c_sh : 0x80000000u;
+            __builtin_amdgcn_raw_buffer_store_b32(w, rs_c, off, 0, 0);
+          } else {
+            u32x2 w;
+            w[0] = pack2<DT>(v[0], v[1]);
+            w[1] = pack2<DT>(v[2], v[3]);
+            const unsigned off = m < p.m ? ((unsigned)m * (unsigned)p.ldc + (unsigned)(n0 + nl)) * 2u + c_sh : 0x80000000u;
+            __builtin_amdgcn_raw_buffer_store_b64(w, rs_c, off, 0, 0);
+          }
+        }
+      }
+      asm volatile("s_waitcnt lgkmcnt(0)" ::: "memory");
+    }
   }
   asm volatile("s_waitcnt vmcnt(0)" ::: "memory");
 }
diff --git a/controlanimate_amd/kernels.py b/controlanimate_amd/kernels.py
--- a/controlanimate_amd/kernels.py
+++ b/controlanimate_amd/kernels.py
@@ -51,7 +51,8 @@
          bias: Optional[torch.Tensor] = None, rowbias: Optional[torch.Tensor] = None,
          rows_per_group: int = 0, residual: Optional[torch.Tensor] = None, alpha: float = 1.0,
          post_scale: float = 1.0, act: int = ACT_NONE, geglu: bool = False, out_f32: bool = False,
-         out: Optional[torch.Tensor] = None, ln=None, row_sums: bool = False) -> torch.Tensor:
+         out: Optional[torch.Tensor] = None, ln=None, row_sums: bool = False, out_reps: int = 1,
+         res_rep_stride: Optional[int] = None) -> torch.Tensor:
     _req_cuda(a, w, a2, bias, rowbias, residual, out)
     assert a.dim() == 2 and a.stride(1) == 1 and w.dim() == 2 and w.is_contiguous()
     m, k1 = a.shape
@@ -62,11 +63,13 @@
     n = w.shape[0]
     assert w.shape[1] == k1 + k2 and w.dtype == a.dtype
     ncols = n // 2 if geglu else n
-    if out is None:
-        out = torch.empty((m, ncols), device=a.device, dtype=torch.float32 if out_f32 else a.dtype)
-    assert out.shape == (m, ncols) and out.stride(1) == 1
+    reps = max(1, int(out_reps))
+    if out is None:
+        out = torch.empty((reps * m, ncols), device=a.device, dtype=torch.float32 if out_f32 else a.dtype)
+    assert out.shape == (reps * m, ncols) and out.stride(1) == 1
     if residual is not None:
-        assert residual.shape == (m, n) and residual.stride(1) == 1 and residual.dtype == a.dtype
+        res_rows = m if (reps == 1 or res_rep_stride == 0) else reps * m
+        assert residual.shape == (res_rows, n) and residual.stride(1) == 1 and residual.dtype == a.dtype
     if bias is not None:
         assert bias.dtype == torch.float32 and bias.numel() == n
     if rowbias is not None:
@@ -78,6 +81,10 @@
                     m=m, n=n, k1=k1, k2=k2, rows_per_group=rows_per_group, alpha=alpha,
                     post_scale=post_scale, act=act, geglu=int(geglu), out_f32=int(out_f32),
                     dtype=dt_code(a.dtype))
+    if reps > 1:
+        args.out_reps, args.c_rep_stride = reps, m * out.stride(0)
+        if residual is not None:
+            args.res_rep_stride = m * residual.stride(0) if res_rep_stride is None else res_rep_stride
     frag = getattr(w, "_frag", None)
     if frag is not None and frag[1] == bool(geglu) and dispatch.gemm_ar:
         args.w_frag = _p(frag[0])
@@ -123,6 +130,24 @@
     return out
 
 
+def gemm_out_reps_supported(a: torch.Tensor, w: torch.Tensor, *, bias: Optional[torch.Tensor] = None, residual: Optional[torch.Tensor] = None,
+                            alpha: float = 1.0, out_reps: int = 2, res_rep_stride: Optional[int] = None) -> bool:
+    m, k1 = a.shape
+    n = w.shape[0]
+    args = GemmArgs(a=_p(a), w=_p(w), c=_p(a), bias=_p(bias), residual=_p(residual), lda=a.stride(0), ldc=n,
+                    ld_res=residual.stride(0) if residual is not None else 0, m=m, n=n, k1=k1, k2=0, alpha=alpha, post_scale=1.0,
+                    dtype=dt_code(a.dtype), out_reps=out_reps, c_rep_stride=m * n)
+    if residual is not None:
+        args.res_rep_stride = m * residual.stride(0) if res_rep_stride is None else res_rep_stride
+    frag = getattr(w, "_frag", None)
+    if frag is not None and not frag[1] and dispatch.gemm_ar:
+        args.w_frag = _p(frag[0])
+    wbytes = int(lib().ca_gemm_workspace_bytes(C.byref(args)))
+    if wbytes > 0:
+        args.workspace, args.workspace_bytes = _p(a), wbytes
+    return bool(lib().ca_gemm_out_reps_supported(C.byref(args)))
+
+
 def attach_w_frag(w: torch.Tensor, geglu: bool = False) -> torch.Tensor:
     _req_cuda(w)
     if w.dim() != 2 or w.shape[1] != 320 or w.shape[0] % 320 != 0 or not w.is_contiguous() or w.dtype not in (torch.float16, torch.bfloat16):
diff --git a/include/controlanimate_hip.h b/include/controlanimate_hip.h
--- a/include/controlanimate_hip.h
+++ b/include/controlanimate_hip.h
@@ -53,8 +53,11 @@
   float* row_sums_out;
   int32_t ln_parts;
   const void* w_frag;
+  int64_t c_rep_stride, res_rep_stride;
+  int32_t out_reps;
 } ca_gemm_args;
 int ca_gemm(const ca_gemm_args* args, void* stream);
+int ca_gemm_out_reps_supported(const ca_gemm_args* args);
 int ca_pack_w_frag(const void* w, int32_t n, int32_t k, int32_t geglu, void* dst, void* stream);
 typedef struct ca_ff_args {
   const void* x;
```

After: 15.97, median of 6. About the same (+0.6%).
